# etri/bwa-mem-scale

Hardware: AMD Instinct MI355X
Metric: Mreads/sec through the GPU hot path (seed -> chain -> extend -> dedup, reads and index resident), 150bp SE vs a synthetic genome of GRCh38 size, at 1 MI355X; % HBM roofline in roofline.frac (higher is better)
Workload: dtype int64 intervals / int16 DP (two columns per register; int32 for queries beyond 191 bases or scores beyond 2^14)

## Files before the change

### bwa-mem-scale_amd/csrc/api_chain.hip

```cpp
#include <cstring>
#include <utility>

#include <rocprim/rocprim.hpp>

#include "stage_state.h"

using namespace bwams;

extern "C" {
int bwams_index_set_contigs(bwams_index_t *ix, const bwams_contig_t *contigs, int32_t n_seqs) {
    if (!ix || !contigs || n_seqs <= 0) return BWAMS_ERR_ARG;
    const int64_t l_pac = (ix->fmi.ref_seq_len - 1) / 2;
    int64_t at = 0;
    for (int32_t i = 0; i < n_seqs; ++i) {
        if (contigs[i].offset != at || contigs[i].len <= 0) {
            set_last_error("bwams_index_set_contigs: sequences must tile [0, l_pac) in order");
            return BWAMS_ERR_ARG;
        }
        at += contigs[i].len;
    }
    if (at != l_pac) {
        set_last_error("bwams_index_set_contigs: sequence lengths do not add up to l_pac");
        return BWAMS_ERR_ARG;
    }
    BWAMS_HIP(hipSetDevice(ix->device));
    BWAMS_HIP(ix->d_contigs.alloc((size_t)n_seqs * sizeof(bwams_contig_t)));
    BWAMS_HIP(hipMemcpy(ix->d_contigs.p, contigs, (size_t)n_seqs * sizeof(bwams_contig_t), hipMemcpyHostToDevice));
    ix->n_seqs = n_seqs;
    return BWAMS_OK;
}

static int flt_chained_seeds(bwams_batch *b, StageState *s, const bwams_mem_opt_t *opt, const DevBns &bns) {
    if (!b->idx->fmi.ref) {
        set_last_error("bwams_chain_run: reads of ~1100 bases and more need the .0123 reference (mem_flt_chained_seeds)");
        return BWAMS_ERR_ARG;
    }
    int mx = -128, mn = 127;
    for (int i = 0; i < 25; ++i) { mx = mx > opt->mat[i] ? mx : opt->mat[i]; mn = mn < opt->mat[i] ? mn : opt->mat[i]; }
    if (mx <= 0 || (opt->o_ins + opt->e_ins) + (opt->o_del + opt->e_del) <= mx - mn) {
        set_last_error("bwams_chain_run: the local SW of mem_flt_chained_seeds needs max(mat) > 0 and oe_ins + oe_del > max(mat) - min(mat)");
        return BWAMS_ERR_UNSUPPORTED;
    }
    hipStream_t st = b->stream;
    const int64_t N = s->ch.n_seeds, N1 = N + 1, C = s->ch.n_chains, n1 = s->ch.nseq + 1;
    BWAMS_HIP(s->ext.cnt.ensure((size_t)N1 * 6 * 4)); BWAMS_HIP(s->ext.ewide.ensure((size_t)(N1 > C + 1 ? N1 : C + 1) * 6 * 8));
    BWAMS_HIP(s->ext.eoffs.ensure((size_t)(N1 > C + 1 ? N1 : C + 1) * 6 * 8)); BWAMS_HIP(s->ch.sw_qb.ensure_n((size_t)N1));
    BWAMS_HIP(s->ch.sw_rb.ensure_n((size_t)N1)); BWAMS_HIP(s->ch.sw_read.ensure_n((size_t)N1)); BWAMS_HIP(s->ch.sw_newn.ensure_n((size_t)(C + 1)));
    BWAMS_HIP(s->ch.seeds2.ensure_n((size_t)N1));
    SeedSwArgs W;
    W.chains = s->ch.chains.p; W.n_chains = C; W.seeds = s->ch.seeds.p; W.n_seeds = N; W.enc = b->d_enc.p; W.cum = b->d_cum.p; W.nseq = s->ch.nseq;
    W.ref = b->idx->fmi.ref; W.bns = bns; W.opt = *opt; W.cnt = s->ext.cnt.as<int32_t>(); W.win_qb = s->ch.sw_qb.p; W.win_rb = s->ch.sw_rb.p;
    W.seed_read = s->ch.sw_read.p;
    launch_seedsw_plan(W, s->ext.ewide.as<int64_t>(), st);
    int rc = scan_rows(b, s->ext.ewide.as<int64_t>(), s->ext.eoffs.as<int64_t>(), 3, N1);
    if (rc) return rc;
    int64_t tot[3];
    for (int r = 0; r < 3; ++r) BWAMS_HIP(hipMemcpyAsync(&tot[r], s->ext.eoffs.as<int64_t>() + r * N1 + N, 8, hipMemcpyDeviceToHost, st));
    BWAMS_HIP(hipStreamSynchronize(st));
    if (tot[1] >= ((int64_t)1 << 31) || tot[2] >= ((int64_t)1 << 31)) {
        set_last_error("bwams_chain_run: seed re-scoring buffers exceed the 31-bit offsets of SeqPair; use smaller chunks");
        return BWAMS_ERR_CAPACITY;
    }
    BWAMS_HIP(s->ext.lpairs.ensure_n((size_t)(tot[0] + 1))); BWAMS_HIP(s->ext.lqer.ensure_n((size_t)tot[1] + 64));
    BWAMS_HIP(s->ext.lref.ensure_n((size_t)tot[2] + 64)); BWAMS_HIP(s->ch.sw_res.ensure_n((size_t)(tot[0] + 1)));
    if (tot[0] > 0) {
        launch_seedsw_build(W, s->ext.eoffs.as<int64_t>(), s->ext.lpairs.p, s->ext.lref.p, s->ext.lqer.p, b->cu_count, st);
        SwParams prm;
        sw_params(*opt, 0, &prm);
        (void)launch_ksw(s->ext.lpairs.p, tot[0], s->ext.lref.p, s->ext.lqer.p, prm, 208, 200, s->ch.sw_res.p, b->d_ctr.p, b->cu_count, st);
    }
    int64_t *cw = s->ext.ewide.as<int64_t>();
    int64_t *coff = s->ext.eoffs.as<int64_t>() + 3 * N1;
    launch_seedsw_apply(W, s->ext.eoffs.as<int64_t>(), s->ch.sw_res.p, s->ch.sw_newn.p, cw, st);
    if ((rc = scan_rows(b, cw, coff, 1, C + 1))) return rc;
    int64_t new_total = 0;
    BWAMS_HIP(hipMemcpyAsync(&new_total, coff + C, 8, hipMemcpyDeviceToHost, st));
    launch_seedsw_repack(W, s->ch.sw_newn.p, coff, s->ch.seeds2.p, s->ch.chain_off.as<int64_t>(), s->ch.chain_off.as<int64_t>() + n1, st);
    BWAMS_HIP(hipStreamSynchronize(st));
    std::swap(s->ch.seeds, s->ch.seeds2);
    s->ch.n_seeds = new_total;
    return BWAMS_OK;
}

struct SeedView {
    const bwams_smem_t *smem;
    int64_t n_smem;
    const int64_t *sa_off, *sa_coord;
    int64_t n_sa;
    bool one_smem_quirk;
};
static int chain_common(bwams_batch *b, const bwams_mem_opt_t *opt, const SeedView &sv, int64_t *n_chains, int64_t *n_seeds);

int bwams_chain_run(bwams_batch_t *b, const bwams_mem_opt_t *opt, int64_t *n_chains, int64_t *n_seeds) {
    if (b && b->stages) b->stages->ch.ran = false;
    if (!b || !b->sd.done || !b->sd.with_sa) {
        set_last_error("bwams_chain_run: run bwams_seed_run(with_sa = 1) first");
        return BWAMS_ERR_ARG;
    }
    int rc = check_opt(opt, "bwams_chain_run");
    if (rc) return rc;
    if ((rc = bwams_seed_counts(b, nullptr, nullptr))) return rc;
    SeedView sv;
    sv.smem = b->sd.d_sorted.p; sv.n_smem = b->sd.n_smem; sv.sa_off = b->sd.d_sa_off.p; sv.sa_coord = b->sd.d_sa_coord.p; sv.n_sa = b->sd.n_sa;
    sv.one_smem_quirk = true;
    return chain_common(b, opt, sv, n_chains, n_seeds);
}

int bwams_chain_run_ert(bwams_batch_t *b, const bwams_mem_opt_t *opt, const bwams_ert_mem_t *mems, const int64_t *mem_off,
                        const uint64_t *hits, const int64_t *hit_off, int64_t *n_chains, int64_t *n_seeds) {
    if (b && b->stages) b->stages->ch.ran = false;
    if (!b || b->nseq <= 0 || !mem_off || !hit_off) {
        set_last_error("bwams_chain_run_ert: upload the reads first (bwams_seed_upload) and pass the MEM / hit offsets");
        return BWAMS_ERR_ARG;
    }
    int rc = check_opt(opt, "bwams_chain_run_ert");
    if (rc) return rc;
    const int64_t nseq = b->nseq, n1 = nseq + 1;
    const int64_t n_mems = mem_off[nseq], n_hits = hit_off[nseq];
    if (mem_off[0] != 0 || hit_off[0] != 0 || n_mems < 0 || n_hits < 0 || (n_mems && !mems) || (n_hits && !hits)) return BWAMS_ERR_ARG;
    for (int64_t r = 0; r < nseq; ++r) {
        if (mem_off[r + 1] < mem_off[r] || hit_off[r + 1] < hit_off[r]) { set_last_error("bwams_chain_run_ert: offsets must be non-decreasing"); return BWAMS_ERR_ARG; }
        const int64_t nh = hit_off[r + 1] - hit_off[r];
        for (int64_t i = mem_off[r]; i < mem_off[r + 1]; ++i) {
            const bwams_ert_mem_t &m = mems[i];
            if (m.start < 0 || m.end <= m.start || m.hitcount < 0 || m.hitbeg < 0 || (int64_t)m.hitbeg + m.hitcount > nh) {
                set_last_error("bwams_chain_run_ert: a MEM with an empty span or a hit slice outside its read's hit array");
                return BWAMS_ERR_ARG;
            }
        }
    }
    BWAMS_HIP(hipSetDevice(b->idx->device));
    StageState *s;
    if ((rc = get_state(b, &s))) return rc;
    hipStream_t st = b->stream;
    BWAMS_HIP(s->ch.et_mems.ensure_n((size_t)(n_mems + 1))); BWAMS_HIP(s->ch.et_moff.ensure_n((size_t)n1));
    BWAMS_HIP(s->ch.et_hoff.ensure_n((size_t)n1)); BWAMS_HIP(s->ch.et_hits.ensure_n((size_t)(n_hits + 1)));
    BWAMS_HIP(s->ch.et_smem.ensure_n((size_t)(n_mems + 1))); BWAMS_HIP(s->ch.et_cnt.ensure_n((size_t)(n_mems + 1)));
    BWAMS_HIP(s->ch.et_off.ensure_n((size_t)(n_mems + 1))); BWAMS_HIP(s->ch.et_srt.ensure((size_t)(n_mems + 1) * 24));
    if (n_mems) BWAMS_HIP(hipMemcpyAsync(s->ch.et_mems.p, mems, (size_t)n_mems * sizeof(bwams_ert_mem_t), hipMemcpyHostToDevice, st));
    if (n_hits) BWAMS_HIP(hipMemcpyAsync(s->ch.et_hits.p, hits, (size_t)n_hits * 8, hipMemcpyHostToDevice, st));
    BWAMS_HIP(hipMemcpyAsync(s->ch.et_moff.p, mem_off, (size_t)n1 * 8, hipMemcpyHostToDevice, st));
    BWAMS_HIP(hipMemcpyAsync(s->ch.et_hoff.p, hit_off, (size_t)n1 * 8, hipMemcpyHostToDevice, st));
    ErtArgs E;
    E.mems = s->ch.et_mems.p; E.mem_off = s->ch.et_moff.p; E.hits = s->ch.et_hits.p; E.hit_off = s->ch.et_hoff.p; E.nseq = nseq; E.n_mems = n_mems;
    E.l_pac = (b->idx->fmi.ref_seq_len - 1) / 2; E.max_occ = opt->max_occ; E.pad_ = 0; E.smem_out = s->ch.et_smem.p; E.cnt = s->ch.et_cnt.p;
    E.srt = s->ch.et_srt.p;
    launch_ert_sort(E, st);
    if ((rc = scan_rows(b, s->ch.et_cnt.p, s->ch.et_off.p, 1, n_mems + 1))) return rc;
    int64_t n_sa = 0;
    BWAMS_HIP(hipMemcpyAsync(&n_sa, s->ch.et_off.p + n_mems, 8, hipMemcpyDeviceToHost, st));
    BWAMS_HIP(hipStreamSynchronize(st));
    BWAMS_HIP(s->ch.et_coord.ensure_n((size_t)(n_sa + 1)));
    launch_ert_pick(E, s->ch.et_off.p, s->ch.et_coord.p, st);
    SeedView sv;
    sv.smem = s->ch.et_smem.p; sv.n_smem = n_mems; sv.sa_off = s->ch.et_off.p;
    sv.sa_coord = s->ch.et_coord.p; sv.n_sa = n_sa; sv.one_smem_quirk = false;
    return chain_common(b, opt, sv, n_chains, n_seeds);
}

static int chain_common(bwams_batch *b, const bwams_mem_opt_t *opt, const SeedView &sv, int64_t *n_chains, int64_t *n_seeds) {
    int rc;
    if (b->max_read_len >= 32768) {
        set_last_error("bwams_chain_run: reads of 32768 bases or more are not supported (16-bit query coordinates)");
        return BWAMS_ERR_UNSUPPORTED;
    }
    BWAMS_HIP(hipSetDevice(b->idx->device));
    StageState *s;
    if ((rc = get_state(b, &s))) return rc;
    outdated(s, From::chain);
    hipStream_t st = b->stream;
    const int64_t nseq = b->nseq, n_sa = sv.n_sa, n1 = nseq + 1;
    const size_t ns = (size_t)(n_sa > 0 ? n_sa : 1);
    BWAMS_HIP(s->ch.s_next.ensure_n(ns)); BWAMS_HIP(s->ch.s_ql.ensure_n(ns)); BWAMS_HIP(s->ch.crec.ensure(chain_rec_bytes(n_sa)));
    BWAMS_HIP(s->ch.flt.ensure_n(ns)); BWAMS_HIP(s->ch.f_rec.ensure_n(ns)); BWAMS_HIP(s->ch.f_first.ensure_n(ns));
    BWAMS_HIP(s->ch.f_kept.ensure_n(ns)); BWAMS_HIP(s->ch.f_sel.ensure_n(ns)); BWAMS_HIP(s->ch.n_chn.ensure_n((size_t)n1));
    BWAMS_HIP(s->heavy.ensure_n((size_t)n1)); BWAMS_HIP(s->ch.redo.ensure_n((size_t)n1)); BWAMS_HIP(s->ch.slice.ensure((size_t)n1 * 16));
    BWAMS_HIP(s->ch.okeys.ensure_n((size_t)n1)); BWAMS_HIP(s->ch.okeys2.ensure_n((size_t)n1)); BWAMS_HIP(s->ch.ovals.ensure_n((size_t)n1));
    BWAMS_HIP(s->ch.ovals2.ensure_n((size_t)n1)); BWAMS_HIP(s->ch.nodes.ensure(chain_node_bytes(n_sa, nseq)));
    BWAMS_HIP(s->ch.n_kept.ensure_n((size_t)n1)); BWAMS_HIP(s->ch.n_kept_seeds.ensure_n((size_t)n1)); BWAMS_HIP(s->ch.read_base.ensure_n((size_t)n1));
    BWAMS_HIP(s->ch.frac.ensure_n((size_t)n1)); BWAMS_HIP(s->ch.wide.ensure((size_t)n1 * 16)); BWAMS_HIP(s->ch.chain_off.ensure((size_t)n1 * 16));

    ChainArgs A;
    A.smem = sv.smem; A.n_smem = sv.n_smem; A.sa_off = sv.sa_off; A.sa_coord = sv.sa_coord; A.cum = b->d_cum.p; A.nseq = nseq;
    if ((rc = dev_bns(b->idx, &A.bns))) return rc;
    A.opt = *opt;
    A.s_next = s->ch.s_next.p; A.s_ql = s->ch.s_ql.p; A.crec = s->ch.crec.p; A.flt = s->ch.flt.p; A.f_rec = s->ch.f_rec.p;
    A.f_first = s->ch.f_first.p; A.f_kept = s->ch.f_kept.p; A.f_sel = s->ch.f_sel.p; A.nodes = s->ch.nodes.p; A.n_kept = s->ch.n_kept.p;
    A.n_kept_seeds = s->ch.n_kept_seeds.p; A.n_chn = s->ch.n_chn.p; A.heavy = s->heavy.p; A.redo = s->ch.redo.p; A.slice = s->ch.slice.as<int64_t>();
    A.order = s->ch.ovals2.p; A.read_base = s->ch.read_base.p; A.frac_rep = s->ch.frac.p; A.ctr = b->d_ctr.p; A.seed_batch = knobs().chain_batch;

    BWAMS_HIP(hipEventRecord(s->ev[0], st));
    static_assert(offsetof(DevCounters, dbg) == offsetof(DevCounters, chain_redo) + 4 * sizeof(unsigned long long), "one memset clears chain_redo .. dbg[18]");
    BWAMS_HIP(hipMemsetAsync(&b->d_ctr.p->chain_redo, 0, 23 * sizeof(unsigned long long), st));
    const bool count_ch = knobs().chain_count != 0;
    if (count_ch) BWAMS_HIP(hipMemsetAsync(b->d_ctr.p->dbg + 61, 0, 4 * sizeof(unsigned long long), st));
    BWAMS_HIP(hipMemsetAsync(&b->d_ctr.p->chain_overflow, 0, 29 * sizeof(unsigned long long), st));
    if ((sv.one_smem_quirk ? sv.n_smem <= 1 : sv.n_smem <= 0) || n_sa == 0) {
        BWAMS_HIP(hipMemsetAsync(s->ch.n_kept.p, 0, (size_t)n1 * 4, st));
        BWAMS_HIP(hipMemsetAsync(s->ch.n_kept_seeds.p, 0, (size_t)n1 * 4, st));
    } else {
        launch_chain_count(A, s->ch.okeys.p, s->ch.ovals.p, st);
        if ((rc = with_tmp(b, "bwams_chain_run: radix_sort_pairs_desc", [&](void *tmp, size_t &tb) {
                return rocprim::radix_sort_pairs_desc(tmp, tb, s->ch.okeys.p, s->ch.okeys2.p, s->ch.ovals.p, s->ch.ovals2.p, (size_t)nseq, 0, 32, st);
            }))) return rc;
        if (launch_chain(A, s->ch.okeys.p, b->cu_count, st, s->aux, s->fork, s->join, count_ch)) {
            set_last_error("bwams_chain_run: stream fork/join failed");
            return BWAMS_ERR_DEVICE;
        }
    }
    int64_t tot[2] = {0, 0};
    if (nseq > 0) {
        launch_widen2(A.n_kept, A.n_kept_seeds, nseq, s->ch.wide.as<int64_t>(), st);
        if ((rc = scan_rows(b, s->ch.wide.as<int64_t>(), s->ch.chain_off.as<int64_t>(), 2, n1))) return rc;
        BWAMS_HIP(hipMemcpyAsync(&tot[0], s->ch.chain_off.as<int64_t>() + nseq, 8, hipMemcpyDeviceToHost, st));
        BWAMS_HIP(hipMemcpyAsync(&tot[1], s->ch.chain_off.as<int64_t>() + n1 + nseq, 8, hipMemcpyDeviceToHost, st));
    } else {
        BWAMS_HIP(hipMemsetAsync(s->ch.chain_off.p, 0, (size_t)n1 * 16, st));
    }
    BWAMS_HIP(hipMemcpyAsync(b->h_ctr.p, b->d_ctr.p, sizeof(DevCounters), hipMemcpyDeviceToHost, st));
    BWAMS_HIP(hipStreamSynchronize(st));
    {
        const bool vb = knobs().verbose != 0;
        if (vb) {
            const unsigned long long *d = b->h_ctr.p->dbg;
            fprintf(stderr, "[bwams_chain_run] filter wave tier: reads by chains <=32 %llu <=64 %llu <=128 %llu <=256 %llu <=512 %llu <=960 %llu more %llu (+ %llu taken sequentially by one lane); "
                            "Mcycles: sequential(HBM) %.1f sort %.1f filter %.1f; chains %llu selected %llu; longest read: sort %.2f filter %.2f Mcycles, most chains %llu, most selected %llu\n",
                    d[0], d[1], d[2], d[3], d[4], d[5], d[6], d[18], d[7] / 1e6, d[8] / 1e6, d[9] / 1e6, d[11], d[10], d[12] / 1e6, d[13] / 1e6, d[14], d[15]);
#ifdef BWAMS_CHAINDBG
            static const char *cn[8] = {"XL", "L", "L2", "L1", "M2", "M", "M1", "S"};
            fprintf(stderr, "[bwams_chain_run] chaining wave tier, per class: reads / mean us / longest us / wave-ms:");
            for (int c = 0; c < 8; ++c) fprintf(stderr, "  %s %llu / %.0f / %.0f / %.1f", cn[c], d[32 + 3 * c], d[32 + 3 * c] ? d[33 + 3 * c] * 1e-2 / d[32 + 3 * c] : 0.0, d[34 + 3 * c] * 1e-2, d[33 + 3 * c] * 1e-5);
            fprintf(stderr, "\n");
            fprintf(stderr, "[bwams_chain_run] wave tier phases, G cycles: preamble %.2f chaining %.2f weights+copy %.2f (sort %.2f filter %.2f: all reads); reads %llu seeds %llu; passes %llu settling %llu seeds (%llu new chains), %llu seeds one by one%s; pass parts, G cycles: batch prologue %.2f search %.2f record+test %.2f settle %.2f commit %.2f one-by-one %.2f\n",
                    d[56] / 1e9, d[57] / 1e9, d[58] / 1e9, d[8] / 1e9, d[9] / 1e9, d[59], d[60], count_ch ? d[61] : 0ull, count_ch ? d[63] : 0ull,
                    count_ch ? d[64] : 0ull, count_ch ? d[62] : 0ull, count_ch ? "" : " (these four are counted under BWAMS_CHAIN_COUNT=1 only)", d[65] / 1e9, d[66] / 1e9, d[67] / 1e9, d[68] / 1e9, d[69] / 1e9, d[70] / 1e9);
#endif
        }
    }
    if (b->h_ctr.p->chain_overflow) {
        set_last_error("bwams_chain_run: internal B-tree node region exhausted");
        return BWAMS_ERR_CAPACITY;
    }
    {
        const DevCounters *h = b->h_ctr.p;
        int64_t *c = s->ch.counts;
        for (int i = 0; i < 10; ++i) c[i] = (int64_t)h->chain_class[i];
        c[10] = (int64_t)h->n_heavy; c[11] = (int64_t)h->chain_redo;
        for (int i = 0; i < 7; ++i) c[12 + i] = (int64_t)h->dbg[i];
        c[19] = (int64_t)h->dbg[18];
        c[20] = count_ch ? (int64_t)h->dbg[16] : -1; c[21] = count_ch ? (int64_t)h->dbg[17] : -1;
        c[22] = count_ch ? (int64_t)h->dbg[61] : -1; c[23] = count_ch ? (int64_t)h->dbg[63] : -1;
        c[24] = count_ch ? (int64_t)h->dbg[64] : -1; c[25] = count_ch ? (int64_t)h->dbg[62] : -1;
        s->ch.ran = true;
    }
    const bool has_long = b->h_ctr.p->chain_longread != 0;
    s->ch.n_redo = (int64_t)b->h_ctr.p->chain_redo;
    s->ch.n_chains = tot[0]; s->ch.n_seeds = tot[1]; s->ch.nseq = nseq;
    BWAMS_HIP(s->ch.chains.ensure_n((size_t)(tot[0] + 1))); BWAMS_HIP(s->ch.seeds.ensure_n((size_t)(tot[1] + 1)));
    if (tot[0] > 0) launch_chain_emit(A, s->ch.chain_off.as<int64_t>(), s->ch.chain_off.as<int64_t>() + n1, s->ch.chains.p, s->ch.seeds.p, st);
    if (has_long && tot[0] > 0 && (rc = flt_chained_seeds(b, s, opt, A.bns))) return rc;
    BWAMS_HIP(hipEventRecord(s->ev[1], st));
    BWAMS_HIP(hipGetLastError());
    s->ch.done = true;
    s->opt = *opt;
    if (n_chains) *n_chains = s->ch.n_chains;
    if (n_seeds) *n_seeds = s->ch.n_seeds;
    return BWAMS_OK;
}

int bwams_chain_fetch(bwams_batch_t *b, bwams_chain_t *chains, int64_t chain_cap, bwams_chain_seed_t *seeds,
                      int64_t seed_cap, int64_t *chain_off) {
    if (!b || !b->stages || !b->stages->ch.done) {
        set_last_error("bwams_chain_fetch: no chains on the device");
        return BWAMS_ERR_ARG;
    }
    StageState *s = b->stages;
    if (s->ch.n_chains > chain_cap || s->ch.n_seeds > seed_cap) return BWAMS_ERR_CAPACITY;
    BWAMS_HIP(hipSetDevice(b->idx->device));
    hipStream_t st = b->stream;
    if (s->ch.n_chains) BWAMS_HIP(hipMemcpyAsync(chains, s->ch.chains.p, (size_t)s->ch.n_chains * sizeof(bwams_chain_t), hipMemcpyDeviceToHost, st));
    if (s->ch.n_seeds) BWAMS_HIP(hipMemcpyAsync(seeds, s->ch.seeds.p, (size_t)s->ch.n_seeds * sizeof(bwams_chain_seed_t), hipMemcpyDeviceToHost, st));
    if (chain_off) BWAMS_HIP(hipMemcpyAsync(chain_off, s->ch.chain_off.p, (size_t)(s->ch.nseq + 1) * 8, hipMemcpyDeviceToHost, st));
    BWAMS_HIP(hipStreamSynchronize(st));
    return BWAMS_OK;
}

int bwams_debug_chain_counts(bwams_batch_t *b, int64_t counts[26]) {
    static_assert(kChainCounts == 26, "include/bwams.h documents 26 counters");
    if (!b || !counts || !b->stages || !b->stages->ch.done || !b->stages->ch.ran) {
        set_last_error("bwams_debug_chain_counts: no bwams_chain_run / bwams_chain_run_ert on this batch");
        return BWAMS_ERR_ARG;
    }
    for (int i = 0; i < kChainCounts; ++i) counts[i] = b->stages->ch.counts[i];
    return BWAMS_OK;
}

int bwams_chain_upload(bwams_batch_t *b, const bwams_chain_t *chains, int64_t n_chains, const bwams_chain_seed_t *seeds,
                       int64_t n_seeds, const int64_t *chain_off) {
    if (!b || !chain_off || n_chains < 0 || n_seeds < 0 || (n_chains && (!chains || !seeds))) return BWAMS_ERR_ARG;
    if (b->nseq <= 0) {
        set_last_error("bwams_chain_upload: upload the reads first (bwams_seed_upload)");
        return BWAMS_ERR_ARG;
    }
    const int64_t nseq = b->nseq, n1 = nseq + 1;
    if (chain_off[0] != 0 || chain_off[nseq] != n_chains) return BWAMS_ERR_ARG;
    int64_t at = 0;
    std::string bad;
    int64_t *soff = new int64_t[(size_t)n1];
    for (int64_t r = 0; r < nseq && bad.empty(); ++r) {
        soff[r] = at;
        if (chain_off[r + 1] < chain_off[r]) bad = "chain_off must be non-decreasing";
        for (int64_t j = chain_off[r]; j < chain_off[r + 1] && bad.empty(); ++j) {
            if (chains[j].seqid != r) bad = "chain.seqid does not match chain_off";
            else if (chains[j].seed_off != at || chains[j].n < 0) bad = "chain.seed_off must enumerate the seed array in order";
            at += chains[j].n;
        }
    }
    soff[nseq] = at;
    if (bad.empty() && at != n_seeds) bad = "seed counts do not add up";
    if (!bad.empty()) {
        delete[] soff;
        set_last_error("bwams_chain_upload: " + bad);
        return BWAMS_ERR_ARG;
    }
    BWAMS_HIP(hipSetDevice(b->idx->device));
    StageState *s;
    int rc = get_state(b, &s);
    if (rc) { delete[] soff; return rc; }
    outdated(s, From::chain);
    hipStream_t st = b->stream;
    BWAMS_HIP(s->ch.chain_off.ensure((size_t)n1 * 16)); BWAMS_HIP(s->ch.chains.ensure_n((size_t)(n_chains + 1)));
    BWAMS_HIP(s->ch.seeds.ensure_n((size_t)(n_seeds + 1)));
    BWAMS_HIP(hipMemcpyAsync(s->ch.chain_off.p, chain_off, (size_t)n1 * 8, hipMemcpyHostToDevice, st));
    BWAMS_HIP(hipMemcpyAsync(s->ch.chain_off.as<int64_t>() + n1, soff, (size_t)n1 * 8, hipMemcpyHostToDevice, st));
    if (n_chains) BWAMS_HIP(hipMemcpyAsync(s->ch.chains.p, chains, (size_t)n_chains * sizeof(bwams_chain_t), hipMemcpyHostToDevice, st));
    if (n_seeds) BWAMS_HIP(hipMemcpyAsync(s->ch.seeds.p, seeds, (size_t)n_seeds * sizeof(bwams_chain_seed_t), hipMemcpyHostToDevice, st));
    BWAMS_HIP(hipStreamSynchronize(st));
    delete[] soff;
    s->ch.n_chains = n_chains; s->ch.n_seeds = n_seeds; s->ch.nseq = nseq;
    s->ch.done = true; s->ch.ran = false;
    return BWAMS_OK;
}
}
```

### bwa-mem-scale_amd/csrc/chain.hip

```cpp
#include "common.h"
#include "chain_kernels.h"
#include "wave_ops.h"
#include "ksort.h"

namespace bwams {
namespace {

constexpr int KB_T = 5;
constexpr int KB_MAXK = 2 * KB_T - 1;
constexpr int kLaneSeeds = 32;
constexpr int kLightChains = 16;
struct alignas(16) Node {
    int16_t n, internal;
    int32_t ptr[KB_MAXK + 1];
    int64_t pos[KB_MAXK];
    int32_t key[KB_MAXK];
};
static_assert(sizeof(Node) == 160, "node layout");

struct alignas(16) ChainRec {
    int64_t last_rbeg, endr;
    uint16_t first_qbeg, last_qbeg, last_len, endq;
    int32_t rid, n;
    int32_t first_idx, last_idx;
    int32_t wq, wr;
};
static_assert(sizeof(ChainRec) == 48, "chain record layout");

__host__ __device__ constexpr size_t lds_bytes(int K) { return (size_t)K * (sizeof(ChainRec) + 12) + 64; }
constexpr int kClassS = 128, kClassM1 = 256, kClassM = 512, kClassL1 = 850, kClassL = 1700;
constexpr int kClassM2 = 665, kClassL2 = 1275;
static_assert(lds_bytes(kClassL) <= 160 * 1024, "class L must fit one CU's LDS");
constexpr int kClassXL = 4096;
constexpr int kClassXL2 = 13000;
__host__ __device__ constexpr size_t lds_bytes_xl(int K) { return (size_t)K * 12 + 64; }

struct RidCache { int64_t lo, hi; int rid; };

__device__ __forceinline__ int pos2rid(const DevBns &b, int64_t pos_f, RidCache &rc) {
    if (pos_f >= b.l_pac) return -1;
    if (pos_f >= rc.lo && pos_f < rc.hi) return rc.rid;
    const int mid = pos2rid(b, pos_f);
    const int64_t off = b.contigs[mid].offset;
    if (pos_f >= off) { rc.lo = off; rc.hi = mid == b.n_seqs - 1 ? b.l_pac : b.contigs[mid + 1].offset; rc.rid = mid; }
    return mid;
}
__device__ __forceinline__ int intv2rid(const DevBns &b, int64_t rb, int64_t re, RidCache &rc) {
    if (rb < b.l_pac && re > b.l_pac) return -2;
    const int rid_b = pos2rid(b, depos(b, rb), rc);
    const int rid_e = rb < re ? pos2rid(b, depos(b, re - 1), rc) : rid_b;
    return rid_b == rid_e ? rid_b : -1;
}

struct WaveBns { int64_t off; };
__device__ __forceinline__ WaveBns wave_bns_load(const DevBns &b, int lane) {
    WaveBns w;
    const int stride = b.n_seqs <= 64 ? 1 : 64;
    const int64_t i = (int64_t)lane * stride;
    w.off = i < b.n_seqs ? b.contigs[i].offset : INT64_MAX;
    return w;
}
__device__ __forceinline__ int pos2rid_w(const DevBns &b, const WaveBns &w, int64_t pos_f, int lane) {
    if (pos_f >= b.l_pac) return -1;
    const int c = __popcll(__ballot(w.off <= pos_f)) - 1;
    if (b.n_seqs <= 64) return c;
    const int i = c * 64 + lane;
    const int64_t o = i < b.n_seqs ? b.contigs[i].offset : INT64_MAX;
    return c * 64 + __popcll(__ballot(o <= pos_f)) - 1;
}
__device__ __forceinline__ int intv2rid_w(const DevBns &b, const WaveBns &w, int64_t rb, int64_t re, int lane) {
    if (rb < b.l_pac && re > b.l_pac) return -2;
    const int rid_b = pos2rid_w(b, w, depos(b, rb), lane);
    const int rid_e = rb < re ? pos2rid_w(b, w, depos(b, re - 1), lane) : rid_b;
    return rid_b == rid_e ? rid_b : -1;
}

struct ReadCtx {
    Node *nodes;
    ChainRec *crec;
    int32_t n_nodes, cap_nodes, root;
    int32_t n_keys;
    bool overflow;
    bool wr;
};

__device__ __forceinline__ int32_t new_node(ReadCtx &c) {
    if (c.n_nodes >= c.cap_nodes) { c.overflow = true; return 0; }
    if (c.wr) { Node *x = &c.nodes[c.n_nodes]; x->n = 0; x->internal = 0; }
    return c.n_nodes++;
}

struct NodeR {
    int32_t n, internal;
    int64_t pos[KB_MAXK];
    int32_t key[KB_MAXK];
    int32_t ptr[KB_MAXK + 1];
};
__device__ __forceinline__ void load_node(const Node *p, NodeR &x, bool want_ptr) {
    x.n = p->n; x.internal = p->internal;
#pragma unroll
    for (int t = 0; t < KB_MAXK; ++t) { x.pos[t] = p->pos[t]; x.key[t] = p->key[t]; }
#pragma unroll
    for (int t = 0; t <= KB_MAXK; ++t) x.ptr[t] = want_ptr ? (int32_t)p->ptr[t] : 0;
}

__device__ __forceinline__ int node_search(const NodeR &x, int64_t k, bool &eq) {
    int cnt = 0;
    bool e = false;
#pragma unroll
    for (int t = 0; t < KB_MAXK; ++t)
        if (t < x.n) { cnt += x.pos[t] < k ? 1 : 0; e |= x.pos[t] == k; }
    eq = e;
    return e ? cnt : cnt - 1;
}
__device__ __forceinline__ int32_t sel_key(const NodeR &x, int i) {
    int32_t v = x.key[0];
#pragma unroll
    for (int t = 1; t < KB_MAXK; ++t) v = i == t ? x.key[t] : v;
    return v;
}
__device__ __forceinline__ int64_t sel_pos(const NodeR &x, int i) {
    int64_t v = x.pos[0];
#pragma unroll
    for (int t = 1; t < KB_MAXK; ++t) v = i == t ? x.pos[t] : v;
    return v;
}
__device__ __forceinline__ int32_t sel_ptr(const NodeR &x, int i) {
    int32_t v = x.ptr[0];
#pragma unroll
    for (int t = 1; t <= KB_MAXK; ++t) v = i == t ? x.ptr[t] : v;
    return v;
}

__device__ __forceinline__ int32_t kbt_lower(const ReadCtx &c, int64_t k, int64_t &lower_pos) {
    int32_t lower = -1, xi = c.root;
    for (;;) {
        NodeR x;
        load_node(&c.nodes[xi], x, true);
        bool eq;
        const int i = node_search(x, k, eq);
        if (i >= 0) { lower = sel_key(x, i); lower_pos = sel_pos(x, i); }
        if (i >= 0 && eq) return lower;
        if (!x.internal) return lower;
        xi = sel_ptr(x, i + 1);
    }
}

__device__ __forceinline__ void kbt_split(ReadCtx &c, int32_t xi, int i, int32_t yi) {
    const int32_t zi = new_node(c);
    if (c.overflow || !c.wr) return;
    Node *x = &c.nodes[xi], *y = &c.nodes[yi], *z = &c.nodes[zi];
    z->internal = y->internal;
    z->n = KB_T - 1;
    for (int t = 0; t < KB_T - 1; ++t) { z->key[t] = y->key[KB_T + t]; z->pos[t] = y->pos[KB_T + t]; }
    if (y->internal) for (int t = 0; t < KB_T; ++t) z->ptr[t] = y->ptr[KB_T + t];
    y->n = KB_T - 1;
    const int xn = x->n;
    for (int t = xn; t > i; --t) x->ptr[t + 1] = x->ptr[t];
    x->ptr[i + 1] = zi;
    for (int t = xn - 1; t >= i; --t) { x->key[t + 1] = x->key[t]; x->pos[t + 1] = x->pos[t]; }
    x->key[i] = y->key[KB_T - 1];
    x->pos[i] = y->pos[KB_T - 1];
    x->n = (int16_t)(xn + 1);
}

__device__ __forceinline__ void kbt_put(ReadCtx &c, int32_t id, int64_t k) {
    ++c.n_keys;
    int32_t xi = c.root;
    if (c.nodes[xi].n == KB_MAXK) {
        const int32_t s = new_node(c);
        if (c.overflow) return;
        if (c.wr) { c.nodes[s].internal = 1; c.nodes[s].n = 0; c.nodes[s].ptr[0] = xi; }
        c.root = s;
        kbt_split(c, s, 0, xi);
        if (c.overflow) return;
        xi = s;
    }
    for (;;) {
        Node *px = &c.nodes[xi];
        NodeR x;
        load_node(px, x, true);
        bool eq;
        if (!x.internal) {
            const int i = node_search(x, k, eq);
            if (c.wr) {
#pragma unroll
                for (int t = KB_MAXK - 1; t >= 1; --t)
                    if (t > i + 1 && t <= x.n) { px->key[t] = x.key[t - 1]; px->pos[t] = x.pos[t - 1]; }
#pragma unroll
                for (int t = 0; t < KB_MAXK; ++t)
                    if (t == i + 1) { px->key[t] = id; px->pos[t] = k; }
                px->n = (int16_t)(x.n + 1);
            }
            return;
        }
        int i = node_search(x, k, eq) + 1;
        int32_t ci = sel_ptr(x, i);
        if (c.nodes[ci].n == KB_MAXK) {
            const int64_t median = c.nodes[ci].pos[KB_T - 1];
            kbt_split(c, xi, i, ci);
            if (c.overflow) return;
            if (k > median) ci = c.nodes[xi].ptr[i + 1];
        }
        xi = ci;
    }
}

struct WPath { int32_t leaf; int16_t slot, n; bool ok; };

__device__ __forceinline__ int32_t kbt_traverse(const ReadCtx &c, int32_t *out) {
    int32_t sx[16];
    int32_t si[16];
    int sp = 0, n = 0;
    sx[0] = c.root; si[0] = 0;
    while (sp >= 0) {
        const Node *x = &c.nodes[sx[sp]];
        if (!x->internal) {
            for (int t = 0; t < x->n; ++t) { if (c.wr) out[n] = x->key[t]; ++n; }
            --sp;
            continue;
        }
        const int i = si[sp];
        if (i > 0 && i - 1 < x->n) { if (c.wr) out[n] = x->key[i - 1]; ++n; }
        if (i <= x->n && sp < 15) {
            si[sp] = i + 1;
            ++sp;
            sx[sp] = x->ptr[i]; si[sp] = 0;
        } else --sp;
    }
    return n;
}

struct FltLt { __device__ __forceinline__ bool operator()(const uint2 &a, const uint2 &b) const { return a.x > b.x; } };

struct FltClose {
    __device__ __forceinline__ void operator()(uint2 *a, int n, void *scratch, int lane, FltLt) const {
        uint2 *out = reinterpret_cast<uint2 *>(scratch);
        if (n > 64) {
            unsigned long long *key = reinterpret_cast<unsigned long long *>(scratch);
            out = reinterpret_cast<uint2 *>(key + n);
            for (int x = lane; x < n; x += 64) key[x] = ((unsigned long long)(0x7fffffffu - a[x].x) << 32) | (unsigned long long)(unsigned)x;
            __syncthreads();
            int P = 128;
            while (P < n) P <<= 1;
            for (int k = 2; k <= P; k <<= 1) {
                for (int j = k >> 1; j > 0; j >>= 1) {
                    const bool flip = j == (k >> 1);
                    for (int c0 = 0; c0 < (P >> 1); c0 += 64) {
                        const int c = c0 + lane;
                        const int i = ((c & ~(j - 1)) << 1) | (c & (j - 1));
                        const int l = flip ? (i ^ (k - 1)) : i + j;
                        if (l < n) {
                            const unsigned long long x = key[i], y = key[l];
                            if (y < x) { key[i] = y; key[l] = x; }
                        }
                    }
                    __syncthreads();
                }
            }
            for (int x = lane; x < n; x += 64) out[x] = a[(uint32_t)key[x]];
            __syncthreads();
        } else {
            const int x = lane;
            const uint2 v = x < n ? a[x] : make_uint2(0u, 0u);
            int pos = 0;
            for (int y = 0; y < n; ++y) {
                const uint32_t wy = a[y].x;
                pos += (wy > v.x || (wy == v.x && y < x)) ? 1 : 0;
            }
            if (x < n) out[pos] = v;
            __syncthreads();
        }
        for (int x = lane; x < n; x += 64) a[x] = out[x];
        __syncthreads();
    }
};

__device__ __forceinline__ void wave_flt_sort(uint2 *a, int n, void *scratch, int lane, int depth0 = 0) {
    wave_ks_introsort(a, n, scratch, reinterpret_cast<int *>(reinterpret_cast<char *>(scratch) + (size_t)n * 8), lane, FltLt(), FltClose(), depth0);
}

__device__ void filter_seq(const bwams_mem_opt_t &opt, int n_chn, uint4 *rec, int32_t *kept, int32_t *sel) {
    int n_sel = 0;
    kept[0] = 3;
    sel[n_sel++] = 0;
    for (int i = 1; i < n_chn; ++i) {
        bool large_ovlp = false;
        const uint4 ri = rec[i];
        const int bi = (int)ri.x, ei = (int)ri.y, wi = (int)(ri.z & 0x7fffffffu);
        const bool alt_i = (ri.z >> 31) != 0;
        int k;
        for (k = 0; k < n_sel; ++k) {
            const int j = sel[k];
            const uint4 rj = rec[j];
            const int bj = (int)rj.x, ej = (int)rj.y;
            const int b_max = bj > bi ? bj : bi;
            const int e_min = ej < ei ? ej : ei;
            const bool alt_j = (rj.z >> 31) != 0;
            if (e_min > b_max && (!alt_j || alt_i)) {
                const int li = ei - bi, lj = ej - bj;
                const int min_l = li < lj ? li : lj;
                if ((float)(e_min - b_max) >= (float)min_l * opt.mask_level && min_l < opt.max_chain_gap) {
                    large_ovlp = true;
                    if ((int)rj.w < 0) rec[j].w = (uint32_t)i;
                    const int wj = (int)(rj.z & 0x7fffffffu);
                    if ((float)wi < (float)wj * opt.drop_ratio && wj - wi >= (opt.min_seed_len << 1)) break;
                }
            }
        }
        if (k == n_sel) {
            sel[n_sel++] = i;
            kept[i] = large_ovlp ? 2 : 3;
        }
    }
    for (int i = 0; i < n_sel; ++i) {
        const int f = (int)rec[sel[i]].w;
        if (f >= 0) kept[f] = 1;
    }
}

__device__ void finish_read(const ChainArgs &A, int64_t r, int64_t base, int n_chn, int L) {
    uint2 *fl = A.flt + base;
    uint4 *rec = A.f_rec + base;
    int32_t *kept = A.f_kept + base, *first = A.f_first + base;
    const ChainRec *crec = reinterpret_cast<const ChainRec *>(A.crec) + base;
    int i, k;
    for (i = k = 0; i < n_chn; ++i) {
        if (kept[i] == 0 || kept[i] == 3) continue;
        if (++k >= A.opt.max_chain_extend) break;
    }
    for (; i < n_chn; ++i)
        if (kept[i] < 3) kept[i] = 0;
    int n_seeds = 0;
    for (i = k = 0; i < n_chn; ++i) {
        if (kept[i] == 0) continue;
        const uint2 f = fl[i];
        const uint32_t alt = rec[i].z & 0x80000000u;
        fl[k] = make_uint2(f.x | ((unsigned)kept[i] << 29) | alt, f.y);
        first[k] = (int32_t)rec[i].w;
        n_seeds += crec[f.y].n;
        ++k;
    }
    A.n_kept[r] = k;
    A.n_kept_seeds[r] = n_seeds;
    if (k) {
        const double min_l = A.opt.min_chain_weight ? (double)(1.1f * (float)A.opt.min_chain_weight) : (double)5.5f * log((double)L);
        if (!(min_l > (double)(0.05f * (float)L))) atomicAdd(&A.ctr->chain_longread, 1ull);
    }
}

__device__ __forceinline__ uint4 make_rec(const ChainArgs &A, const ChainRec &c, uint32_t w) {
    const uint32_t alt = A.bns.contigs[c.rid].is_alt != 0 ? 0x80000000u : 0u;
    return make_uint4((uint32_t)c.first_qbeg, (uint32_t)(c.last_qbeg + c.last_len), w | alt, 0xffffffffu);
}

#ifndef BWAMS_CHAIN_COUNT_TU
__global__ void chain_slice_kernel(ChainArgs A) {
    const int64_t i = (int64_t)blockIdx.x * blockDim.x + threadIdx.x;
    if (i >= A.n_smem) return;
    const int64_t r = (int64_t)A.smem[i].rid;
    if (i == 0 || (int64_t)A.smem[i - 1].rid != r) A.slice[2 * r] = i;
    if (i + 1 == A.n_smem || (int64_t)A.smem[i + 1].rid != r) A.slice[2 * r + 1] = i + 1;
}
__global__ void chain_count_kernel(ChainArgs A, uint32_t *keys, uint32_t *vals) {
    const int64_t r = (int64_t)blockIdx.x * blockDim.x + threadIdx.x;
    const bool live = r < A.nseq;
    int64_t cnt = 0;
    if (live) {
        const int64_t beg = A.slice[2 * r], end = A.slice[2 * r + 1];
        cnt = beg < end ? A.sa_off[end] - A.sa_off[beg] : 0;
        keys[r] = (uint32_t)(cnt < 0xffffffffll ? cnt : 0xffffffffll);
        vals[r] = (uint32_t)r;
    }
    const int thr[10] = {kClassL, kClassL1, kClassM, kClassM1, kClassS, kLaneSeeds, kClassXL, kClassL2, kClassM2, kClassXL2};
    if (!__ballot(live && cnt > kLaneSeeds)) return;
#pragma unroll
    for (int c = 0; c < 10; ++c) {
        const unsigned long long m = __ballot(live && cnt > thr[c]);
        if (m && (threadIdx.x & 63) == 0) atomicAdd(&A.ctr->chain_class[c], (unsigned long long)__popcll(m));
    }
}

#endif

__device__ __forceinline__ int sarr_lower(const int64_t *key, int n, int64_t k, int lane, bool &eq) {
    int base = 0;
    if (n > 4096) {
        const int nsc = (n + 4095) >> 12;
        const unsigned long long ms = __ballot(lane < nsc && key[lane << 12] <= k);
        if (!ms) { eq = false; return -1; }
        base = (__popcll(ms) - 1) << 12;
        key += base;
        n = n - base < 4096 ? n - base : 4096;
    }
    const int nch = (n + 63) >> 6;
    const unsigned long long mc = __ballot(lane < nch && key[lane << 6] <= k);
    if (!mc) { eq = false; return -1; }
    const int c = __popcll(mc) - 1;
    const int i = (c << 6) + lane;
    const int64_t my = i < n ? key[i] : 0;
    const unsigned long long mk = __ballot(i < n && my <= k);
    const int idx = base + (c << 6) + __popcll(mk) - 1;
    eq = __ballot(i < n && my == k) != 0;
    return idx;
}
__device__ __forceinline__ void sarr_insert(int64_t *key, int32_t *cid, int n, int at, int64_t k, int32_t id, int lane) {
    for (int base = ((n - at) >> 6) << 6; base >= 0; base -= 64) {
        const int i = at + base + lane;
        const bool mv = i < n;
        const int64_t kk = mv ? key[i] : 0;
        const int32_t cc = mv ? cid[i] : 0;
        if (mv) { key[i + 1] = kk; cid[i + 1] = cc; }
    }
    if (lane == 0) { key[at] = k; cid[at] = id; }
}

struct SeedCtx {
    bool crec_hbm;
    const int64_t *pos;
    int32_t *s_next;
    int2 *s_ql;
    ChainRec *crec;
    int64_t *s_key;
    int32_t *s_cid;
};
__device__ __forceinline__ bool chain_seed_one(const ChainArgs &A, const SeedCtx &S, int &n_keys, int32_t g, int64_t rbeg, int rid, int qbeg,
                                               int slen, int lane) {
    const bool wr = lane == 0;
    const int64_t l_pac = A.bns.l_pac;
    bool to_add = true, eq = false;
    int idx = -1;
    if (n_keys) {
        idx = sarr_lower(S.s_key, n_keys, rbeg, lane, eq);
        if (idx >= 0) {
            const int32_t lower = S.s_cid[idx];
            const int64_t fr = S.s_key[idx];
            ChainRec ch = S.crec[lower];
            const int64_t lr = ch.last_rbeg;
            const int64_t qend = ch.last_qbeg + ch.last_len, rend = lr + ch.last_len;
            if (rid != ch.rid) to_add = true;
            else if (qbeg >= ch.first_qbeg && qbeg + slen <= qend && rbeg >= fr && rbeg + slen <= rend) to_add = false;
            else if ((lr < l_pac || fr < l_pac) && rbeg >= l_pac) to_add = true;
            else {
                const int64_t x = qbeg - ch.last_qbeg, y = rbeg - lr;
                if (y >= 0 && x - y <= A.opt.w && y - x <= A.opt.w && x - ch.last_len < A.opt.max_chain_gap && y - ch.last_len < A.opt.max_chain_gap) {
                    if (wr) { S.s_ql[g] = make_int2(qbeg, slen); S.s_next[g] = -1; S.s_next[ch.last_idx] = g; }
                    if (qbeg >= ch.endq) ch.wq += slen; else if (qbeg + slen > ch.endq) ch.wq += qbeg + slen - ch.endq;
                    ch.endq = (uint16_t)((int)ch.endq > qbeg + slen ? (int)ch.endq : qbeg + slen);
                    if (rbeg >= ch.endr) ch.wr += slen; else if (rbeg + slen > ch.endr) ch.wr += (int)(rbeg + slen - ch.endr);
                    ch.endr = ch.endr > rbeg + slen ? ch.endr : rbeg + slen;
                    ch.last_rbeg = rbeg; ch.last_qbeg = (uint16_t)qbeg; ch.last_len = (uint16_t)slen; ch.last_idx = g; ch.n += 1;
                    if (wr) S.crec[lower] = ch;
                    to_add = false;
                }
            }
        }
    }
    if (to_add) {
        if (n_keys && eq) return false;
        if (wr) {
            S.s_ql[g] = make_int2(qbeg, slen); S.s_next[g] = -1;
            ChainRec ch;
            ch.last_rbeg = rbeg; ch.endr = rbeg + slen;
            ch.first_qbeg = (uint16_t)qbeg; ch.last_qbeg = (uint16_t)qbeg; ch.last_len = (uint16_t)slen; ch.endq = (uint16_t)(qbeg + slen);
            ch.rid = rid; ch.n = 1; ch.first_idx = g; ch.last_idx = g; ch.wq = slen; ch.wr = slen;
            S.crec[n_keys] = ch;
        }
        sarr_insert(S.s_key, S.s_cid, n_keys, n_keys ? idx + 1 : 0, rbeg, n_keys, lane);
        ++n_keys;
    }
    return true;
}
template <bool COUNT>
__device__ bool chain_seeds_batch(const ChainArgs &A, const SeedCtx &S, int &n_keys, const bwams_smem_t *sm, int64_t beg, int64_t end, int64_t base,
                                  int32_t cnt, RidCache &rc, const WaveBns &wb, int lane) {
    enum { NONE = 0, NOOP = 1, MERGE = 2, NEW = 3, UNSETTLED = 4 };
    const int64_t l_pac = A.bns.l_pac;
    const unsigned long long below = (1ull << lane) - 1ull;
    const int w = A.opt.w, max_gap = A.opt.max_chain_gap;
    int64_t i_lo = beg;
#ifdef BWAMS_CHAINDBG
    unsigned long long tq[6] = {0, 0, 0, 0, 0, 0};
    unsigned long long tq0 = __builtin_amdgcn_s_memtime();
#define TQ(k) { const unsigned long long t_ = __builtin_amdgcn_s_memtime(); tq[k] += t_ - tq0; tq0 = t_; }
#else
#define TQ(k)
#endif
    const int nsm = (int)(end - beg);
    const bool sm_regs = nsm <= 64;
    int sm_start = INT32_MAX, sm_q = 0, sm_l = 0;
    if (sm_regs && lane < nsm) {
        sm_start = (int)(A.sa_off[beg + lane] - base);
        sm_q = (int)sm[beg + lane].m; sm_l = (int)sm[beg + lane].n + 1 - sm_q;
    }
    for (int32_t gb = 0; gb < cnt; gb += 64) {
        const int32_t g = gb + lane;
        bool pend = g < cnt;
        const int64_t rbeg = pend ? S.pos[g] : 0;
        int qbeg = 0, slen = 0;
        if (sm_regs) {
            int k = 0;
            for (int i = 0; i < nsm; ++i) k += __builtin_amdgcn_readlane(sm_start, i) <= g ? 1 : 0;
            const int src = k > 0 ? k - 1 : 0;
            qbeg = __shfl(sm_q, src); slen = __shfl(sm_l, src);
        } else {
            int64_t lo = i_lo, hi = end - 1;
            if (pend) {
                while (lo < hi) {
                    const int64_t mid = (lo + hi + 1) >> 1;
                    if (A.sa_off[mid] - base <= g) lo = mid; else hi = mid - 1;
                }
                qbeg = (int)sm[lo].m; slen = (int)sm[lo].n + 1 - qbeg;
            }
            i_lo = readlane64(lo, 0);
        }
        int rid = -1;
        if (A.bns.n_seqs <= 64) {
            const int64_t rb = rbeg, re = rbeg + slen;
            const int64_t pb = depos(A.bns, rb), pe = rb < re ? depos(A.bns, re - 1) : pb;
            int cb = 0, ce = 0;
            for (int i = 0; i < A.bns.n_seqs; ++i) {
                const int64_t o = readlane64(wb.off, i);
                cb += o <= pb ? 1 : 0; ce += o <= pe ? 1 : 0;
            }
            rid = (rb < l_pac && re > l_pac) ? -2 : cb == ce ? cb - 1 : -1;
        } else if (pend) rid = intv2rid(A.bns, rbeg, rbeg + slen, rc);
        pend = pend && rid >= 0;
        int one_by_one = 0;
        unsigned long long mp;
        TQ(0)
        while ((mp = __ballot(pend)) != 0ull) {
            if (one_by_one) {
                const int l0 = __builtin_ctzll(mp);
                if (!chain_seed_one(A, S, n_keys, gb + l0, readlane64(rbeg, l0), __builtin_amdgcn_readlane(rid, l0), __builtin_amdgcn_readlane(qbeg, l0),
                                    __builtin_amdgcn_readlane(slen, l0), lane)) return false;
                if (lane == l0) pend = false;
                if constexpr (COUNT) { if (lane == 0) atomicAdd(&A.ctr->dbg[62], 1ull); }
                --one_by_one;
                TQ(5)
                continue;
            }
            const int n = n_keys;
            int idx = -1;
            if (n) {
                int step = 1;
                while ((step << 1) <= n) step <<= 1;
                for (; step > 0; step >>= 1) {
                    const int t = idx + step;
                    if (pend && t < n && S.s_key[t] <= rbeg) idx = t;
                }
            }
            TQ(1)
            int64_t lo_key = INT64_MIN;
            int32_t lower = -1;
            int act = NONE;
            ChainRec ch;
            ch.last_rbeg = 0; ch.endr = 0; ch.first_qbeg = ch.last_qbeg = ch.last_len = ch.endq = 0; ch.rid = ch.n = ch.first_idx = ch.last_idx = ch.wq = ch.wr = 0;
            if (pend) {
                act = NEW;
                if (idx >= 0) {
                    lo_key = S.s_key[idx];
                    lower = S.s_cid[idx];
                    ch = S.crec[lower];
                    const int64_t lr = ch.last_rbeg;
                    const int64_t qend = ch.last_qbeg + ch.last_len, rend = lr + ch.last_len;
                    if (rid != ch.rid) act = NEW;
                    else if (qbeg >= ch.first_qbeg && qbeg + slen <= qend && rbeg >= lo_key && rbeg + slen <= rend) act = NOOP;
                    else if ((lr < l_pac || lo_key < l_pac) && rbeg >= l_pac) act = NEW;
                    else {
                        const int64_t x = qbeg - ch.last_qbeg, y = rbeg - lr;
                        if (y >= 0 && x - y <= w && y - x <= w && x - ch.last_len < max_gap && y - ch.last_len < max_gap) act = MERGE;
                    }
                }
            }
            const bool eq = pend && idx >= 0 && lo_key == rbeg;
            TQ(2)
            int64_t best = lo_key;
            int best_rid = -1, best_q = 0, best_l = 0;
            bool displaced = false, touched = false;
            int first_open = 64;
            bool shared = false;
            {
                unsigned *mark = reinterpret_cast<unsigned *>(S.s_cid);
                const bool in_arr = pend && idx >= 0;
                if (in_arr) atomicAdd(&mark[idx], 1u << 24);
                if (in_arr) shared = (mark[idx] >> 24) > 1u;
                if (in_arr) atomicSub(&mark[idx], 1u << 24);
                const bool under = pend && idx < 0;
                const int n_under = __popcll(__ballot(under));
                if (under && n_under > 1) shared = true;
            }
            unsigned long long rem = __ballot(pend && shared);
            while (rem) {
                const int i = __builtin_ctzll(rem);
                rem &= rem - 1;
                int fin = act;
                if (displaced) {
                    const int64_t x = qbeg - best_q, y = rbeg - best;
                    if (rid != best_rid) fin = NEW;
                    else if (qbeg >= best_q && qbeg + slen <= best_q + best_l && rbeg + slen <= best + best_l) fin = NOOP;
                    else if (best < l_pac && rbeg >= l_pac) fin = NEW;
                    else fin = (x - y <= w && y - x <= w && x - best_l < max_gap && y - best_l < max_gap) ? UNSETTLED : NEW;
                } else if (touched) fin = UNSETTLED;
                const int a_i = __builtin_amdgcn_readlane(fin, i);
                if (a_i == UNSETTLED) { first_open = i; break; }
                if (lane == i) act = fin;
                if (a_i == NEW) {
                    const int64_t rb_i = readlane64(rbeg, i);
                    const int rid_i = __builtin_amdgcn_readlane(rid, i), q_i = __builtin_amdgcn_readlane(qbeg, i), l_i = __builtin_amdgcn_readlane(slen, i);
                    if (lane > i && rb_i <= rbeg && rb_i > best) { best = rb_i; best_rid = rid_i; best_q = q_i; best_l = l_i; displaced = true; }
                } else if (a_i == MERGE) {
                    const int low_i = __builtin_amdgcn_readlane(lower, i);
                    if (lane > i && lower == low_i) touched = true;
                }
            }
            const bool com = pend && lane < first_open;
            TQ(3)
            const unsigned long long m_new = __ballot(com && act == NEW);
            if (__ballot(com && act == NEW && (eq || (displaced && best == rbeg)))) return false;
            if (com && act == MERGE) {
                S.s_ql[g] = make_int2(qbeg, slen); S.s_next[g] = -1; S.s_next[ch.last_idx] = g;
                if (qbeg >= ch.endq) ch.wq += slen; else if (qbeg + slen > ch.endq) ch.wq += qbeg + slen - ch.endq;
                ch.endq = (uint16_t)((int)ch.endq > qbeg + slen ? (int)ch.endq : qbeg + slen);
                if (rbeg >= ch.endr) ch.wr += slen; else if (rbeg + slen > ch.endr) ch.wr += (int)(rbeg + slen - ch.endr);
                ch.endr = ch.endr > rbeg + slen ? ch.endr : rbeg + slen;
                ch.last_rbeg = rbeg; ch.last_qbeg = (uint16_t)qbeg; ch.last_len = (uint16_t)slen; ch.last_idx = g; ch.n += 1;
                S.crec[lower] = ch;
            }
            if (m_new) {
                const int m = __popcll(m_new);
                const bool mine = com && act == NEW;
                int min_idx = mine ? idx : n;
                for (int d = 32; d >= 1; d >>= 1) { const int o = __shfl_xor(min_idx, d); min_idx = o < min_idx ? o : min_idx; }
                for (int cb = n > 0 ? ((n - 1) >> 6) << 6 : -64; cb >= 0 && cb + 63 > min_idx; cb -= 64) {
                    const int p = cb + lane;
                    const bool mv = p < n;
                    const int64_t kk = mv ? S.s_key[p] : 0;
                    const int32_t cc = mv ? S.s_cid[p] : 0;
                    int sh = __popcll(__ballot(mine && idx < cb));
                    unsigned long long mm = __ballot(mine && idx >= cb && idx < cb + 64);
                    while (mm) { const int i = __builtin_ctzll(mm); mm &= mm - 1; sh += __builtin_amdgcn_readlane(idx, i) < p ? 1 : 0; }
                    if (mv && sh) { S.s_key[p + sh] = kk; S.s_cid[p + sh] = cc; }
                }
                int rank = 0;
                { unsigned long long mm = m_new; while (mm) { const int i = __builtin_ctzll(mm); mm &= mm - 1; rank += __builtin_amdgcn_readlane(idx, i) < idx ? 1 : 0; } }
                { unsigned long long mm = m_new & __ballot(shared); while (mm) { const int i = __builtin_ctzll(mm); mm &= mm - 1; rank += (__builtin_amdgcn_readlane(idx, i) == idx && readlane64(rbeg, i) < rbeg) ? 1 : 0; } }
                if (mine) {
                    const int32_t cid = n + __popcll(m_new & below);
                    S.s_ql[g] = make_int2(qbeg, slen); S.s_next[g] = -1;
                    ChainRec nc;
                    nc.last_rbeg = rbeg; nc.endr = rbeg + slen;
                    nc.first_qbeg = (uint16_t)qbeg; nc.last_qbeg = (uint16_t)qbeg; nc.last_len = (uint16_t)slen; nc.endq = (uint16_t)(qbeg + slen);
                    nc.rid = rid; nc.n = 1; nc.first_idx = g; nc.last_idx = g; nc.wq = slen; nc.wr = slen;
                    S.crec[cid] = nc;
                    S.s_key[idx + 1 + rank] = rbeg; S.s_cid[idx + 1 + rank] = cid;
                }
                n_keys = n + m;
            }
            if (com) pend = false;
            if constexpr (COUNT) {
                const unsigned long long n_com = (unsigned long long)__popcll(__ballot(com));
                if (lane == 0) { atomicAdd(&A.ctr->dbg[61], 1ull); atomicAdd(&A.ctr->dbg[63], n_com); atomicAdd(&A.ctr->dbg[64], (unsigned long long)__popcll(m_new)); }
            }
            if (__popcll(__ballot(com)) <= 1) one_by_one = 8;
            if (S.crec_hbm) __threadfence_block();
            TQ(4)
        }
    }
#ifdef BWAMS_CHAINDBG
    if (lane == 0) for (int k = 0; k < 6; ++k) atomicAdd(&A.ctr->dbg[65 + k], tq[k]);
#endif
    return true;
}

__device__ void heavy_read(const ChainArgs &A, int64_t r, int64_t base, int n_chn, unsigned char *lds, int cap, int lane);
__host__ __device__ constexpr size_t heavy_lds_bytes(int cap);
template <bool LDS, int CONT = 0, bool CREC_HBM = false, bool COUNT = false>
__device__ __forceinline__ bool chain_read(const ChainArgs &A, int64_t r, int lane, int nl, Node *nodes, int32_t cap_nodes,
                                           ChainRec *crec_w, int32_t cap_chains) {
    const bool wr = lane == 0;
#ifdef BWAMS_CHAINDBG
    const unsigned long long tp0 = __builtin_amdgcn_s_memtime();
#endif
    if (wr) {
        A.n_kept[r] = 0;
        A.n_kept_seeds[r] = 0;
        A.read_base[r] = 0;
        A.n_chn[r] = 0;
    }
    const bwams_smem_t *sm = A.smem;
    const int64_t beg = A.slice[2 * r], end = A.slice[2 * r + 1];
    const int L = (int)(A.cum[r + 1] - A.cum[r]);
    if (beg == end || L < A.opt.min_seed_len) return true;

    int b = 0, e = 0, l_rep = 0;
    if (nl == 64 && end - beg <= 64) {
        const bool has = beg + lane < end;
        const int my_b = has ? (int)sm[beg + lane].m : 0, my_e = has ? (int)sm[beg + lane].n + 1 : 0;
        unsigned long long rep = __ballot(has && sm[beg + lane].s > (int64_t)A.opt.max_occ);
        while (rep) {
            const int i = __builtin_ctzll(rep);
            rep &= rep - 1;
            const int sb = __builtin_amdgcn_readlane(my_b, i), se = __builtin_amdgcn_readlane(my_e, i);
            if (sb > e) { l_rep += e - b; b = sb; e = se; }
            else e = e > se ? e : se;
        }
    } else
    for (int64_t i = beg; i < end; ++i) {
        const int sb = (int)sm[i].m, se = (int)sm[i].n + 1;
        if (sm[i].s <= (int64_t)A.opt.max_occ) continue;
        if (sb > e) { l_rep += e - b; b = sb; e = se; }
        else e = e > se ? e : se;
    }
    l_rep += e - b;
    if (wr) A.frac_rep[r] = (float)l_rep / (float)L;

    const int64_t base = A.sa_off[beg];
    const int32_t cnt = (int32_t)(A.sa_off[end] - base);
    if (wr) A.read_base[r] = base;
    if (cnt == 0) return true;
    const int64_t *pos = A.sa_coord + base;
    int32_t *s_next = A.s_next + base;
    int2 *s_ql = A.s_ql + base;
    ChainRec *crec_g = reinterpret_cast<ChainRec *>(A.crec) + base;
    ChainRec *crec;
    ReadCtx c;
    if constexpr (LDS) {
        crec = CREC_HBM ? crec_g : crec_w;
        c.nodes = nodes; c.cap_nodes = cap_nodes;
    } else {
        crec = crec_g;
        const int64_t nbase = (base >> 1) + 2 * r;
        c.nodes = reinterpret_cast<Node *>(A.nodes) + nbase;
        c.cap_nodes = (int32_t)((((base + cnt) >> 1) + 2 * (r + 1)) - nbase);
    }
    c.crec = crec;
    c.n_nodes = 0; c.n_keys = 0; c.overflow = false; c.wr = wr;
    int64_t *s_key = nullptr;
    int32_t *s_cid = nullptr;
    if constexpr (CONT == 1) {
        s_key = reinterpret_cast<int64_t *>(nodes);
        s_cid = reinterpret_cast<int32_t *>(s_key + cap_chains);
    } else c.root = new_node(c);
    RidCache rc;
    rc.lo = 0; rc.hi = -1; rc.rid = 0;
    WaveBns wb;
    wb.off = 0;
    if (nl == 64 && A.bns.n_seqs <= 4096) wb = wave_bns_load(A.bns, lane);
    if (LDS && cnt > cap_chains) { if (wr) atomicAdd(&A.ctr->chain_overflow, 1ull); return true; }

    const int64_t l_pac = A.bns.l_pac;
#ifdef BWAMS_CHAINDBG
    const unsigned long long tp1 = __builtin_amdgcn_s_memtime();
#endif
    if constexpr (CONT == 1) {
        if (nl == 64 && A.seed_batch) {
            SeedCtx S;
            S.pos = pos; S.s_next = s_next; S.s_ql = s_ql; S.crec = crec; S.s_key = s_key; S.s_cid = s_cid; S.crec_hbm = CREC_HBM;
            int nk = 0;
            if (!chain_seeds_batch<COUNT>(A, S, nk, sm, beg, end, base, cnt, rc, wb, lane)) return false;
            c.n_keys = nk;
        }
    }
    if (!(CONT == 1 && nl == 64 && A.seed_batch))
    for (int64_t i = beg; i < end; ++i) {
        const int qbeg = (int)sm[i].m, slen = (int)sm[i].n + 1 - (int)sm[i].m;
        const int32_t g0 = (int32_t)(A.sa_off[i] - base), g1 = (int32_t)(A.sa_off[i + 1] - base);
        int64_t pos64 = 0;
        for (int32_t g = g0; g < g1; ++g) {
            int64_t rbeg;
            if (nl == 64) {
                const int j = (g - g0) & 63;
                if (j == 0) pos64 = g + lane < g1 ? pos[g + lane] : 0;
                rbeg = (int64_t)(((unsigned long long)(uint32_t)__builtin_amdgcn_readlane((int)(pos64 >> 32), j) << 32) |
                                 (unsigned long long)(uint32_t)__builtin_amdgcn_readlane((int)pos64, j));
            } else rbeg = pos[g];
            const int rid = nl == 64 && A.bns.n_seqs <= 4096 ? intv2rid_w(A.bns, wb, rbeg, rbeg + slen, lane)
                                                               : intv2rid(A.bns, rbeg, rbeg + slen, rc);
            if (rid < 0) continue;
            bool to_add = true;
            WPath path;
            path.ok = false;
            if (c.n_keys) {
                int64_t fr = 0;
                int32_t lower;
                if constexpr (CONT == 1) {
                    bool eq;
                    const int idx = sarr_lower(s_key, c.n_keys, rbeg, lane, eq);
                    lower = -1;
                    if (idx >= 0) { lower = s_cid[idx]; fr = s_key[idx]; }
                    path.slot = (int16_t)0; path.leaf = idx; path.ok = !eq;
                } else lower = kbt_lower(c, rbeg, fr);
                if (lower >= 0) {
                    ChainRec ch = crec[lower];
                    const int64_t lr = ch.last_rbeg;
                    const int64_t qend = ch.last_qbeg + ch.last_len, rend = lr + ch.last_len;
                    if (rid != ch.rid) to_add = true;
                    else if (qbeg >= ch.first_qbeg && qbeg + slen <= qend && rbeg >= fr && rbeg + slen <= rend) to_add = false;
                    else if ((lr < l_pac || fr < l_pac) && rbeg >= l_pac) to_add = true;
                    else {
                        const int64_t x = qbeg - ch.last_qbeg, y = rbeg - lr;
                        if (y >= 0 && x - y <= A.opt.w && y - x <= A.opt.w && x - ch.last_len < A.opt.max_chain_gap &&
                            y - ch.last_len < A.opt.max_chain_gap) {
                            if (wr) {
                                s_ql[g] = make_int2(qbeg, slen);
                                s_next[g] = -1;
                                s_next[ch.last_idx] = g;
                            }
                            if (qbeg >= ch.endq) ch.wq += slen; else if (qbeg + slen > ch.endq) ch.wq += qbeg + slen - ch.endq;
                            ch.endq = (uint16_t)((int)ch.endq > qbeg + slen ? (int)ch.endq : qbeg + slen);
                            if (rbeg >= ch.endr) ch.wr += slen; else if (rbeg + slen > ch.endr) ch.wr += (int)(rbeg + slen - ch.endr);
                            ch.endr = ch.endr > rbeg + slen ? ch.endr : rbeg + slen;
                            ch.last_rbeg = rbeg; ch.last_qbeg = (uint16_t)qbeg; ch.last_len = (uint16_t)slen; ch.last_idx = g; ch.n += 1;
                            if (wr) crec[lower] = ch;
                            to_add = false;
                        }
                    }
                }
            }
            if (to_add) {
                if (wr) { s_ql[g] = make_int2(qbeg, slen); s_next[g] = -1; }
                ChainRec ch;
                ch.last_rbeg = rbeg; ch.endr = rbeg + slen;
                ch.first_qbeg = (uint16_t)qbeg; ch.last_qbeg = (uint16_t)qbeg; ch.last_len = (uint16_t)slen; ch.endq = (uint16_t)(qbeg + slen);
                ch.rid = rid; ch.n = 1; ch.first_idx = g; ch.last_idx = g; ch.wq = slen; ch.wr = slen;
                const int32_t cid = c.n_keys;
                if (wr) crec[cid] = ch;
                if constexpr (CONT == 1) {
                    if (c.n_keys && !path.ok) return false;
                    sarr_insert(s_key, s_cid, c.n_keys, c.n_keys ? path.leaf + 1 : 0, rbeg, cid, lane);
                    ++c.n_keys;
                } else kbt_put(c, cid, rbeg);
                if (c.overflow) { if (wr) atomicAdd(&A.ctr->chain_overflow, 1ull); return true; }
            }
        }
    }
    if (c.n_keys == 0) return true;
#ifdef BWAMS_CHAINDBG
    const unsigned long long tp2 = __builtin_amdgcn_s_memtime();
#endif

    int32_t *ord = A.f_first + base;
    int32_t n_trav;
    if constexpr (CONT == 1) {
        n_trav = c.n_keys;
        for (int32_t t = lane; t < n_trav; t += nl) ord[t] = s_cid[t];
        __threadfence_block();
    } else n_trav = kbt_traverse(c, ord);
    uint2 *fl = A.flt + base;
    int n_chn = 0;
    if (nl == 64) {
        uint2 first = make_uint2(0u, 0u);
        for (int32_t t0 = 0; t0 < n_trav; t0 += 64) {
            const int32_t t = t0 + lane;
            const bool ok = t < n_trav;
            int32_t id = 0;
            if (ok) { if constexpr (CONT == 1) id = s_cid[t]; else id = ord[t]; }
            const ChainRec *pc = &crec[id];
            int w = pc->wr < pc->wq ? pc->wr : pc->wq;
            w = w < (1 << 30) ? w : (1 << 30) - 1;
            if (t0 == 0) first = make_uint2((unsigned)__builtin_amdgcn_readfirstlane(w), (unsigned)__builtin_amdgcn_readfirstlane(id));
            const bool keep = ok && w >= A.opt.min_chain_weight;
            const unsigned long long m = __ballot(keep);
            if (keep) fl[n_chn + __popcll(m & ((1ull << lane) - 1ull))] = make_uint2((unsigned)w, (unsigned)id);
            n_chn += __popcll(m);
        }
        if (n_chn == 0 && wr) fl[0] = first;
        __threadfence_block();
    } else
    for (int32_t t = 0; t < n_trav; ++t) {
        const int32_t id = ord[t];
        const ChainRec ch = crec[id];
        int w = ch.wr < ch.wq ? ch.wr : ch.wq;
        w = w < (1 << 30) ? w : (1 << 30) - 1;
        if (t == 0 && wr) fl[0] = make_uint2((unsigned)w, (unsigned)id);
        if (w < A.opt.min_chain_weight) continue;
        if (wr) fl[n_chn] = make_uint2((unsigned)w, (unsigned)id);
        ++n_chn;
    }
    if (n_chn == 0) n_chn = 1;
    if constexpr (LDS && !CREC_HBM)
        for (int32_t k = lane; k < c.n_keys; k += nl) crec_g[k] = crec_w[k];
    if constexpr (LDS) {
        if (nl == 64) {
#ifdef BWAMS_CHAINDBG
            if (wr) {
                const unsigned long long tp3 = __builtin_amdgcn_s_memtime();
                atomicAdd(&A.ctr->dbg[56], tp1 - tp0); atomicAdd(&A.ctr->dbg[57], tp2 - tp1); atomicAdd(&A.ctr->dbg[58], tp3 - tp2);
                atomicAdd(&A.ctr->dbg[59], 1ull); atomicAdd(&A.ctr->dbg[60], (unsigned long long)cnt);
            }
#endif
            unsigned char *region = CREC_HBM ? reinterpret_cast<unsigned char *>(nodes) : reinterpret_cast<unsigned char *>(crec_w);
            const size_t bytes = (size_t)cap_chains * (CREC_HBM ? 12 : sizeof(ChainRec) + 12);
            const int cap_f = (int)((bytes - 64) / 41);
            if (cap_f >= 64 && n_chn <= cap_f) {
                if (wr) A.n_chn[r] = n_chn;
                __threadfence_block();
                if constexpr (COUNT) { if (wr) atomicAdd(&A.ctr->dbg[16], 1ull); }
                heavy_read(A, r, base, n_chn, region, cap_f, lane);
                return true;
            }
        }
    }
    if (!wr) return true;
    A.n_chn[r] = n_chn;
    if (n_chn > kLightChains) {
        const unsigned long long slot = atomicAdd(&A.ctr->n_heavy, 1ull);
        A.heavy[slot] = (int32_t)r;
        return true;
    }
    if constexpr (COUNT) atomicAdd(&A.ctr->dbg[17], 1ull);
    ks_introsort(fl, n_chn, FltLt());
    uint4 *rec = A.f_rec + base;
    int32_t *kept = A.f_kept + base;
    for (int i = 0; i < n_chn; ++i) {
        rec[i] = make_rec(A, crec[fl[i].y], fl[i].x);
        kept[i] = 0;
    }
    filter_seq(A.opt, n_chn, rec, kept, A.f_sel + base);
    if constexpr (LDS) __threadfence_block();
    finish_read(A, r, base, n_chn, L);
    return true;
}

template <bool COUNT>
__global__ __launch_bounds__(64) void chain_kernel(ChainArgs A, const uint32_t *__restrict__ n_seeds) {
    const int64_t r = (int64_t)blockIdx.x * blockDim.x + threadIdx.x;
    if (r >= A.nseq) return;
    if (n_seeds[r] > (uint32_t)kLaneSeeds) return;
    chain_read<false, 0, false, COUNT>(A, r, 0, 1, nullptr, 0, nullptr, 0);
}

template <bool COUNT>
__global__ __launch_bounds__(64) __attribute__((amdgpu_waves_per_eu(3, 3))) void chain_wave_kernel(ChainArgs A, const unsigned long long *lo_p, const unsigned long long *hi_p,
                                                        unsigned long long *ticket, int K) {
    extern __shared__ __align__(16) unsigned char l_mem[];
    const int lane = threadIdx.x;
    const int64_t lo = lo_p ? (int64_t)*lo_p : 0, hi = (int64_t)*hi_p;
    ChainRec *l_crec = reinterpret_cast<ChainRec *>(l_mem);
    Node *l_nodes = reinterpret_cast<Node *>(l_mem + (size_t)(K > 0 ? K : 0) * sizeof(ChainRec));
    for (;;) {
        const unsigned long long t = wave_ticket(ticket, 1ull);
        if (lo + (int64_t)t >= hi) break;
        const int64_t r = (int64_t)A.order[lo + (int64_t)t];
#ifdef BWAMS_CHAINDBG
        const unsigned long long tk0 = wall_clock64();
#endif
        if (K < 0) {
            if (!chain_read<true, 1, true, COUNT>(A, r, lane, 64, reinterpret_cast<Node *>(l_mem), 0, nullptr, -K) && lane == 0)
                A.redo[atomicAdd(&A.ctr->chain_redo, 1ull)] = (int32_t)r;
        } else if (K) {
            if (!chain_read<true, 1, false, COUNT>(A, r, lane, 64, l_nodes, 0, l_crec, K) && lane == 0)
                A.redo[atomicAdd(&A.ctr->chain_redo, 1ull)] = (int32_t)r;
        } else chain_read<false, 0, false, COUNT>(A, r, lane, 64, nullptr, 0, nullptr, 0);
        __syncthreads();
#ifdef BWAMS_CHAINDBG
        if (lane == 0) {
            const int c = K < 0 ? 0 : K == kClassL ? 1 : K == kClassL2 ? 2 : K == kClassL1 ? 3 : K == kClassM2 ? 4 : K == kClassM ? 5 : K == kClassM1 ? 6 : 7;
            const unsigned long long dt = wall_clock64() - tk0;
            atomicAdd(&A.ctr->dbg[32 + 3 * c], 1ull); atomicAdd(&A.ctr->dbg[33 + 3 * c], dt); atomicMax(&A.ctr->dbg[34 + 3 * c], dt);
        }
#endif
    }
}

template <bool COUNT>
__global__ __launch_bounds__(64) void chain_redo_kernel(ChainArgs A) {
    const int lane = threadIdx.x;
    const int64_t n = (int64_t)A.ctr->chain_redo;
    for (;;) {
        const int64_t t = (int64_t)wave_ticket(&A.ctr->chain_redo_ticket, 1ull);
        if (t >= n) break;
        chain_read<false, 0, false, COUNT>(A, A.redo[t], lane, 64, nullptr, 0, nullptr, 0);
    }
}

constexpr int kHeavyCap[6] = {64, 128, 256, 512, 960, 3840};
__host__ __device__ constexpr size_t heavy_lds_bytes(int cap) { return (size_t)cap * 41 + 64; }
static_assert(heavy_lds_bytes(kHeavyCap[5]) <= 160 * 1024, "the largest class must fit one CU's LDS");
static_assert(160 * 1024 / 41 <= 65535, "wave_ks_introsort's stopper lists are uint16_t: no LDS class may hold more chains");

__device__ void heavy_read(const ChainArgs &A, int64_t r, int64_t base, int n_chn, unsigned char *lds, int cap, int lane) {
    uint4 *l_rec = reinterpret_cast<uint4 *>(lds);
    uint4 *l_sel = l_rec + cap;
    uint2 *l_fl = reinterpret_cast<uint2 *>(l_sel + cap);
    uint8_t *l_kept = reinterpret_cast<uint8_t *>(l_fl + cap);
    const int L = (int)(A.cum[r + 1] - A.cum[r]);
    uint2 *fl = A.flt + base;
    const ChainRec *crec = reinterpret_cast<const ChainRec *>(A.crec) + base;
    const unsigned long long t_0 = __builtin_amdgcn_s_memtime();
    if (lane == 0) {
        const int bk = n_chn <= 32 ? 0 : n_chn <= 64 ? 1 : n_chn <= 128 ? 2 : n_chn <= 256 ? 3 : n_chn <= 512 ? 4 : n_chn <= 960 ? 5 : 6;
        atomicAdd(&A.ctr->dbg[bk], 1ull);
    }
    {
        __syncthreads();
        for (int i = lane; i < n_chn; i += 64) l_fl[i] = fl[i];
        __syncthreads();
        wave_flt_sort(l_fl, n_chn, l_sel, lane);
        const unsigned long long t_1 = __builtin_amdgcn_s_memtime();
        for (int i = lane; i < n_chn; i += 64) {
            const uint2 f = l_fl[i];
            l_rec[i] = make_rec(A, crec[f.y], f.x);
            l_kept[i] = 0;
        }
        __syncthreads();
        int n_sel = 1;
        if (lane == 0) { const uint4 r0 = l_rec[0]; l_sel[0] = make_uint4(r0.x, r0.y, r0.z, 0u); l_kept[0] = 3; }
        __syncthreads();
        const float mask_level = A.opt.mask_level, drop_ratio = A.opt.drop_ratio;
        const int max_gap = A.opt.max_chain_gap, min_dw = A.opt.min_seed_len << 1;
        for (int ib = 1; ib < n_chn; ib += 64) {
            const int i = ib + lane;
            const bool valid = i < n_chn;
            const uint4 ri = valid ? l_rec[i] : make_uint4(0, 0, 0, 0);
            const int bi = (int)ri.x, ei = (int)ri.y, wi = (int)(ri.z & 0x7fffffffu), li = ei - bi;
            const bool alt_i = (ri.z >> 31) != 0;
            const float fwi = (float)wi;
            bool alive = valid, large = false;
            const int n_sel0 = n_sel;
            for (int k0 = 0; k0 < n_sel0; k0 += 4) {
                uint4 rj[4];
#pragma unroll
                for (int u = 0; u < 4; ++u) rj[u] = l_sel[k0 + u < n_sel0 ? k0 + u : n_sel0 - 1];
#pragma unroll
                for (int u = 0; u < 4; ++u) {
                    if (k0 + u >= n_sel0) break;
                    const int bj = (int)rj[u].x, ej = (int)rj[u].y;
                    const int b_max = bj > bi ? bj : bi, e_min = ej < ei ? ej : ei;
                    const bool alt_j = (rj[u].z >> 31) != 0;
                    const int lj = ej - bj, min_l = li < lj ? li : lj;
                    const bool lg = alive && e_min > b_max && (!alt_j || alt_i) && (float)(e_min - b_max) >= (float)min_l * mask_level && min_l < max_gap;
                    const unsigned long long m_lg = __ballot(lg);
                    if (m_lg) {
                        if (lane == __builtin_ctzll(m_lg)) atomicMin(&l_rec[rj[u].w].w, (uint32_t)i);
                        if (lg) {
                            large = true;
                            const int wj = (int)(rj[u].z & 0x7fffffffu);
                            if (fwi < (float)wj * drop_ratio && wj - wi >= min_dw) alive = false;
                        }
                    }
                }
                if (!__ballot(alive)) break;
            }
            unsigned long long todo = __ballot(alive);
            while (todo) {
                const int lp = __builtin_ctzll(todo);
                const int bj = __builtin_amdgcn_readlane(bi, lp), ej = __builtin_amdgcn_readlane(ei, lp);
                const uint32_t zj = (uint32_t)__builtin_amdgcn_readlane((int)ri.z, lp);
                if (lane == lp) { l_sel[n_sel] = make_uint4(ri.x, ri.y, ri.z, (uint32_t)i); l_kept[i] = large ? 2 : 3; }
                ++n_sel;
                const int b_max = bj > bi ? bj : bi, e_min = ej < ei ? ej : ei;
                const bool alt_j = (zj >> 31) != 0;
                const int lj = ej - bj, min_l = li < lj ? li : lj;
                const bool lg = alive && lane > lp && e_min > b_max && (!alt_j || alt_i) && (float)(e_min - b_max) >= (float)min_l * mask_level && min_l < max_gap;
                const unsigned long long m_lg = __ballot(lg);
                if (m_lg) {
                    if (lane == __builtin_ctzll(m_lg)) l_rec[ib + lp].w = (uint32_t)i;
                    if (lg) {
                        large = true;
                        const int wj = (int)(zj & 0x7fffffffu);
                        if (fwi < (float)wj * drop_ratio && wj - wi >= min_dw) alive = false;
                    }
                }
                todo = __ballot(alive) & ~((2ull << lp) - 1ull);
            }
            __syncthreads();
        }
        for (int k = lane; k < n_sel; k += 64) {
            const int f = (int)l_rec[l_sel[k].w].w;
            if (f >= 0) l_kept[f] = 1;
        }
        __syncthreads();
        if (lane == 0) {
            const unsigned long long t_2 = __builtin_amdgcn_s_memtime();
            atomicAdd(&A.ctr->dbg[8], t_1 - t_0);
            atomicAdd(&A.ctr->dbg[9], t_2 - t_1);
            atomicMax(&A.ctr->dbg[12], t_1 - t_0);
            atomicMax(&A.ctr->dbg[13], t_2 - t_1);
            atomicMax(&A.ctr->dbg[14], (unsigned long long)n_chn);
            atomicMax(&A.ctr->dbg[15], (unsigned long long)n_sel);
            atomicAdd(&A.ctr->dbg[10], (unsigned long long)n_sel);
            atomicAdd(&A.ctr->dbg[11], (unsigned long long)n_chn);
        }
        if (A.opt.max_chain_extend <= n_chn) {
            if (lane == 0) {
                int i, k;
                for (i = k = 0; i < n_chn; ++i) {
                    if (l_kept[i] == 0 || l_kept[i] == 3) continue;
                    if (++k >= A.opt.max_chain_extend) break;
                }
                for (; i < n_chn; ++i)
                    if (l_kept[i] < 3) l_kept[i] = 0;
            }
            __syncthreads();
        }
        int32_t *first = A.f_first + base;
        int n_out = 0, n_seeds = 0;
        for (int ib = 0; ib < n_chn; ib += 64) {
            const int i = ib + lane;
            const int kp = i < n_chn ? (int)l_kept[i] : 0;
            const unsigned long long m = __ballot(kp != 0);
            if (kp) {
                const int o = n_out + __popcll(m & ((1ull << lane) - 1ull));
                const uint2 f = l_fl[i];
                const uint4 rc4 = l_rec[i];
                fl[o] = make_uint2(f.x | ((unsigned)kp << 29) | (rc4.z & 0x80000000u), f.y);
                first[o] = (int32_t)rc4.w;
                n_seeds += crec[f.y].n;
            }
            n_out += __popcll(m);
        }
        for (int d = 32; d >= 1; d >>= 1) n_seeds += __shfl_xor(n_seeds, d);
        if (lane == 0) {
            A.n_kept[r] = n_out;
            A.n_kept_seeds[r] = n_seeds;
            if (n_out) {
                const double min_l = A.opt.min_chain_weight ? (double)(1.1f * (float)A.opt.min_chain_weight) : (double)5.5f * log((double)L);
                if (!(min_l > (double)(0.05f * (float)L))) atomicAdd(&A.ctr->chain_longread, 1ull);
            }
        }
        __syncthreads();
    }
}

__global__ __launch_bounds__(64) void chain_heavy_kernel(ChainArgs A, const unsigned long long *n_heavy_p, int cap_lo, int cap,
                                                         unsigned long long *ticket) {
    extern __shared__ __align__(16) unsigned char l_heavy[];
    const int kLdsChains = cap;
    const int lane = threadIdx.x;
    const int64_t n_heavy = (int64_t)*n_heavy_p;
    for (;;) {
        const int64_t hi = (int64_t)wave_ticket(ticket, 1ull);
        if (hi >= n_heavy) break;
        const int64_t r = A.heavy[hi];
        const int64_t base = A.read_base[r];
        const int n_chn = A.n_chn[r];
        if (n_chn <= cap_lo || (n_chn > cap && cap != kHeavyCap[5])) continue;
        const int L = (int)(A.cum[r + 1] - A.cum[r]);
        uint2 *fl = A.flt + base;
        uint4 *rec = A.f_rec + base;
        int32_t *kept = A.f_kept + base;
        const ChainRec *crec = reinterpret_cast<const ChainRec *>(A.crec) + base;
        if (n_chn > kLdsChains) {
            const unsigned long long t_0 = __builtin_amdgcn_s_memtime();
            if (lane == 0) {
                atomicAdd(&A.ctr->dbg[18], 1ull);
                ks_introsort(fl, n_chn, FltLt());
                for (int i = 0; i < n_chn; ++i) { rec[i] = make_rec(A, crec[fl[i].y], fl[i].x); kept[i] = 0; }
                filter_seq(A.opt, n_chn, rec, kept, A.f_sel + base);
                finish_read(A, r, base, n_chn, L);
                atomicAdd(&A.ctr->dbg[7], __builtin_amdgcn_s_memtime() - t_0);
            }
            continue;
        }
        heavy_read(A, r, base, n_chn, l_heavy, cap, lane);
    }
}

#ifndef BWAMS_CHAIN_COUNT_TU
__global__ __launch_bounds__(256) void chain_emit_kernel(ChainArgs A, const int64_t *__restrict__ chain_off, const int64_t *__restrict__ seed_off,
                                                         bwams_chain_t *chains, bwams_chain_seed_t *seeds) {
    const int64_t r = ((int64_t)blockIdx.x * blockDim.x + threadIdx.x) >> 4;
    const int sub = threadIdx.x & 15;
    const bool live = r < A.nseq;
    const int nk = live ? A.n_kept[r] : 0;
    if (nk == 0) return;
    const int64_t base = A.read_base[r];
    const uint2 *fl = A.flt + base;
    const int32_t *first = A.f_first + base;
    const int32_t *s_next = A.s_next + base;
    const int2 *s_ql = A.s_ql + base;
    const int64_t *pos = A.sa_coord + base;
    const ChainRec *crec = reinterpret_cast<const ChainRec *>(A.crec) + base;
    int64_t so0 = seed_off[r];
    const int64_t co = chain_off[r];
    const float frac = A.frac_rep[r];
    for (int j0 = 0; j0 < nk; j0 += 16) {
        const int j = j0 + sub;
        const bool has = j < nk;
        uint2 f = make_uint2(0u, 0u);
        ChainRec ch;
        ch.n = 0; ch.first_idx = -1; ch.rid = 0;
        if (has) { f = fl[j]; ch = crec[f.y]; }
        const int n = has ? ch.n : 0;
        int incl = n;
        for (int d = 1; d < 16; d <<= 1) {
            const int o = __shfl_up(incl, d, 16);
            if (sub >= d) incl += o;
        }
        const int total = __shfl(incl, 15, 16);
        if (has) {
            int64_t so = so0 + (incl - n);
            bwams_chain_t c;
            c.seqid = (int32_t)r; c.cseed = 0;
            c.n = n;
            int m = 1;
            while (m < n) m <<= 1;
            c.m = m;
            c.first = first[j];
            c.rid = ch.rid;
            c.w_kept_alt = f.x;
            c.frac_rep = frac;
            c.pos = pos[ch.first_idx];
            c.seed_off = so;
            chains[co + j] = c;
            for (int32_t g = ch.first_idx; g >= 0; g = s_next[g]) {
                bwams_chain_seed_t sd;
                sd.rbeg = pos[g];
                sd.qbeg = s_ql[g].x; sd.len = s_ql[g].y; sd.score = sd.len;
                sd.done = 0; sd.pad0_[0] = sd.pad0_[1] = sd.pad0_[2] = 0;
                sd.aln = 0; sd.pad1_ = 0;
                seeds[so++] = sd;
            }
        }
        so0 += total;
    }
}

constexpr int kFltTestN = 1024;
__global__ __launch_bounds__(64) void flt_sort_test_kernel(const uint2 *__restrict__ in, int n, int mode, int32_t *__restrict__ order,
                                                           uint2 *__restrict__ scratch) {
    __shared__ uint2 l_a[kFltTestN];
    __shared__ uint4 l_scr[kFltTestN];
    const int lane = threadIdx.x;
    if (mode == 2 || mode == 4) {
        for (int i = lane; i < n; i += 64) scratch[i] = in[i];
        __syncthreads();
        if (lane == 0) ks_introsort(scratch, n, FltLt(), mode == 4 ? 2 : 0);
        __syncthreads();
        for (int i = lane; i < n; i += 64) order[i] = (int32_t)scratch[i].y;
        return;
    }
    for (int i = lane; i < n; i += 64) l_a[i] = in[i];
    __syncthreads();
    wave_flt_sort(l_a, n, l_scr, lane, mode == 3 ? 2 : 0);
    for (int i = lane; i < n; i += 64) order[i] = (int32_t)l_a[i].y;
}

#endif

}

#ifndef BWAMS_CHAIN_COUNT_TU
size_t chain_node_bytes(int64_t n_sa, int64_t nseq) { return (size_t)((n_sa >> 1) + 2 * nseq + 4) * sizeof(Node); }
size_t chain_rec_bytes(int64_t n_sa) { return (size_t)(n_sa > 0 ? n_sa : 1) * sizeof(ChainRec); }

void launch_chain_count(const ChainArgs &A, uint32_t *keys, uint32_t *vals, hipStream_t st) {
    if (A.nseq <= 0) return;
    (void)hipMemsetAsync(A.slice, 0, (size_t)A.nseq * 16, st);
    if (A.n_smem > 0) chain_slice_kernel<<<(unsigned)((A.n_smem + 255) / 256), 256, 0, st>>>(A);
    chain_count_kernel<<<(unsigned)((A.nseq + 255) / 256), 256, 0, st>>>(A, keys, vals);
}
#endif
template <bool COUNT>
static int launch_chain_t(const ChainArgs &A, const uint32_t *n_seeds, int cu_count, hipStream_t st, hipStream_t *aux,
                          hipEvent_t fork, hipEvent_t *join) {
    if (A.nseq <= 0) return 0;
    unsigned long long *cls = A.ctr->chain_class, *tk = A.ctr->chain_ticket;
    if (hipFuncSetAttribute(reinterpret_cast<const void *>(chain_wave_kernel<COUNT>), hipFuncAttributeMaxDynamicSharedMemorySize,
                            (int)lds_bytes_xl(kClassXL2)) != hipSuccess) return -1;
    if (hipEventRecord(fork, st) != hipSuccess) return -1;
    for (int i = 0; i < 7; ++i)
        if (hipStreamWaitEvent(aux[i], fork, 0) != hipSuccess) return -1;
    chain_wave_kernel<COUNT><<<(unsigned)cu_count, 64, lds_bytes_xl(kClassXL2), st>>>(A, cls + 9, cls + 6, tk + 9, -kClassXL2);
    chain_wave_kernel<COUNT><<<(unsigned)(cu_count * 8), 64, 0, aux[0]>>>(A, nullptr, cls + 9, tk + 0, 0);
    chain_wave_kernel<COUNT><<<(unsigned)cu_count, 64, lds_bytes_xl(kClassXL), aux[0]>>>(A, cls + 6, cls + 0, tk + 6, -kClassXL);
    chain_wave_kernel<COUNT><<<(unsigned)cu_count, 64, lds_bytes(kClassL), aux[1]>>>(A, cls + 0, cls + 7, tk + 1, kClassL);
    chain_wave_kernel<COUNT><<<(unsigned)(cu_count * 2), 64, lds_bytes(kClassL2), aux[5]>>>(A, cls + 7, cls + 1, tk + 7, kClassL2);
    chain_wave_kernel<COUNT><<<(unsigned)(cu_count * 3), 64, lds_bytes(kClassL1), aux[2]>>>(A, cls + 1, cls + 8, tk + 2, kClassL1);
    chain_wave_kernel<COUNT><<<(unsigned)(cu_count * 4), 64, lds_bytes(kClassM2), aux[6]>>>(A, cls + 8, cls + 2, tk + 8, kClassM2);
    chain_wave_kernel<COUNT><<<(unsigned)(cu_count * 8), 64, lds_bytes(kClassM1), aux[2]>>>(A, cls + 3, cls + 4, tk + 4, kClassM1);
    chain_wave_kernel<COUNT><<<(unsigned)(cu_count * 12), 64, lds_bytes(kClassS), aux[3]>>>(A, cls + 4, cls + 5, tk + 5, kClassS);
    chain_kernel<COUNT><<<(unsigned)((A.nseq + 63) / 64), 64, 0, aux[1]>>>(A, n_seeds);
    chain_wave_kernel<COUNT><<<(unsigned)(cu_count * 5), 64, lds_bytes(kClassM), aux[5]>>>(A, cls + 2, cls + 3, tk + 3, kClassM);
    for (int i = 0; i < 7; ++i) {
        if (hipEventRecord(join[i], aux[i]) != hipSuccess) return -1;
        if (hipStreamWaitEvent(st, join[i], 0) != hipSuccess) return -1;
    }
    chain_redo_kernel<COUNT><<<(unsigned)(cu_count * 2), 64, 0, st>>>(A);
    if (hipFuncSetAttribute(reinterpret_cast<const void *>(chain_heavy_kernel), hipFuncAttributeMaxDynamicSharedMemorySize,
                            (int)heavy_lds_bytes(kHeavyCap[5])) != hipSuccess) return -1;
    if (hipEventRecord(fork, st) != hipSuccess) return -1;
    for (int i = 0; i < 5; ++i)
        if (hipStreamWaitEvent(aux[i], fork, 0) != hipSuccess) return -1;
    unsigned long long *htk = A.ctr->heavy_tickets;
    chain_heavy_kernel<<<(unsigned)cu_count, 64, heavy_lds_bytes(kHeavyCap[5]), st>>>(A, &A.ctr->n_heavy, kHeavyCap[4], kHeavyCap[5], htk + 5);
    chain_heavy_kernel<<<(unsigned)(cu_count * 4), 64, heavy_lds_bytes(kHeavyCap[4]), aux[1]>>>(A, &A.ctr->n_heavy, kHeavyCap[3], kHeavyCap[4], htk + 4);
    chain_heavy_kernel<<<(unsigned)(cu_count * 7), 64, heavy_lds_bytes(kHeavyCap[3]), aux[2]>>>(A, &A.ctr->n_heavy, kHeavyCap[2], kHeavyCap[3], htk + 3);
    chain_heavy_kernel<<<(unsigned)(cu_count * 12), 64, heavy_lds_bytes(kHeavyCap[2]), aux[0]>>>(A, &A.ctr->n_heavy, kHeavyCap[1], kHeavyCap[2], htk + 2);
    chain_heavy_kernel<<<(unsigned)(cu_count * 16), 64, heavy_lds_bytes(kHeavyCap[1]), aux[3]>>>(A, &A.ctr->n_heavy, kHeavyCap[0], kHeavyCap[1], htk + 1);
    chain_heavy_kernel<<<(unsigned)(cu_count * 24), 64, heavy_lds_bytes(kHeavyCap[0]), aux[4]>>>(A, &A.ctr->n_heavy, 0, kHeavyCap[0], htk + 0);
    for (int i = 0; i < 5; ++i) {
        if (hipEventRecord(join[i], aux[i]) != hipSuccess) return -1;
        if (hipStreamWaitEvent(st, join[i], 0) != hipSuccess) return -1;
    }
    return 0;
}
#ifdef BWAMS_CHAIN_COUNT_TU
int launch_chain_counting(const ChainArgs &A, const uint32_t *n_seeds, int cu_count, hipStream_t st, hipStream_t *aux, hipEvent_t fork, hipEvent_t *join) {
    return launch_chain_t<true>(A, n_seeds, cu_count, st, aux, fork, join);
}
#else
int launch_chain_counting(const ChainArgs &A, const uint32_t *n_seeds, int cu_count, hipStream_t st, hipStream_t *aux, hipEvent_t fork, hipEvent_t *join);
int launch_chain(const ChainArgs &A, const uint32_t *n_seeds, int cu_count, hipStream_t st, hipStream_t *aux,
                 hipEvent_t fork, hipEvent_t *join, bool count) {
    return count ? launch_chain_counting(A, n_seeds, cu_count, st, aux, fork, join) : launch_chain_t<false>(A, n_seeds, cu_count, st, aux, fork, join);
}
void launch_chain_emit(const ChainArgs &A, const int64_t *chain_off, const int64_t *seed_off, bwams_chain_t *chains,
                       bwams_chain_seed_t *seeds, hipStream_t st) {
    if (A.nseq <= 0) return;
    chain_emit_kernel<<<(unsigned)((A.nseq * 16 + 255) / 256), 256, 0, st>>>(A, chain_off, seed_off, chains, seeds);
}

int launch_flt_sort_test(const int64_t *w, int n, int mode, int32_t *order) {
    if (n < 0 || n > kFltTestN) return -1;
    std::vector<uint2> h((size_t)n + 1);
    for (int i = 0; i < n; ++i) h[i] = make_uint2((unsigned)w[i], (unsigned)i);
    DevBuf<uint2> d_in, d_scr;
    DevBuf<int32_t> d_ord;
    if (d_in.alloc(8 * (size_t)(n + 1)) != hipSuccess || d_scr.alloc(8 * (size_t)(n + 1)) != hipSuccess || d_ord.alloc(4 * (size_t)(n + 1)) != hipSuccess ||
        hipMemcpy(d_in.p, h.data(), 8 * (size_t)n, hipMemcpyHostToDevice) != hipSuccess) return -1;
    flt_sort_test_kernel<<<1, 64>>>(d_in.p, n, mode, d_ord.p, d_scr.p);
    if (hipDeviceSynchronize() != hipSuccess || hipMemcpy(order, d_ord.p, 4 * (size_t)n, hipMemcpyDeviceToHost) != hipSuccess) return -1;
    return 0;
}
#endif

}
```

Before: 10.43.

## Replace sorted chain-key array with pre-ranked seeds and LDS occupancy bitmap

Before chaining, the seeds of each read are ranked by reference position with an in-LDS bitonic sort. Chain lookup becomes a predecessor query on a two-level occupancy bitmap indexed by seed rank, replacing the binary search and shift-insert into a sorted key array. Weight extraction now walks the bitmap in rank order instead of reading a sorted cid array. This trades per-insert O(n) shifts for an upfront sort per read plus extra LDS for the bitmap, which may lower occupancy for the larger classes.

```diff
diff --git a/bwa-mem-scale_amd/csrc/api_chain.hip b/bwa-mem-scale_amd/csrc/api_chain.hip
--- a/bwa-mem-scale_amd/csrc/api_chain.hip
+++ b/bwa-mem-scale_amd/csrc/api_chain.hip
@@ -194,6 +194,10 @@
     BWAMS_HIP(hipMemsetAsync(&b->d_ctr.p->chain_redo, 0, 23 * sizeof(unsigned long long), st));
     const bool count_ch = knobs().chain_count != 0;
     if (count_ch) BWAMS_HIP(hipMemsetAsync(b->d_ctr.p->dbg + 61, 0, 4 * sizeof(unsigned long long), st));
+#ifdef BWAMS_CHAINDBG
+    BWAMS_HIP(hipMemsetAsync(b->d_ctr.p->dbg + 32, 0, 29 * sizeof(unsigned long long), st));
+    BWAMS_HIP(hipMemsetAsync(b->d_ctr.p->dbg + 65, 0, 7 * sizeof(unsigned long long), st));
+#endif
     BWAMS_HIP(hipMemsetAsync(&b->d_ctr.p->chain_overflow, 0, 29 * sizeof(unsigned long long), st));
     if ((sv.one_smem_quirk ? sv.n_smem <= 1 : sv.n_smem <= 0) || n_sa == 0) {
         BWAMS_HIP(hipMemsetAsync(s->ch.n_kept.p, 0, (size_t)n1 * 4, st));
@@ -231,8 +235,8 @@
             fprintf(stderr, "[bwams_chain_run] chaining wave tier, per class: reads / mean us / longest us / wave-ms:");
             for (int c = 0; c < 8; ++c) fprintf(stderr, "  %s %llu / %.0f / %.0f / %.1f", cn[c], d[32 + 3 * c], d[32 + 3 * c] ? d[33 + 3 * c] * 1e-2 / d[32 + 3 * c] : 0.0, d[34 + 3 * c] * 1e-2, d[33 + 3 * c] * 1e-5);
             fprintf(stderr, "\n");
-            fprintf(stderr, "[bwams_chain_run] wave tier phases, G cycles: preamble %.2f chaining %.2f weights+copy %.2f (sort %.2f filter %.2f: all reads); reads %llu seeds %llu; passes %llu settling %llu seeds (%llu new chains), %llu seeds one by one%s; pass parts, G cycles: batch prologue %.2f search %.2f record+test %.2f settle %.2f commit %.2f one-by-one %.2f\n",
-                    d[56] / 1e9, d[57] / 1e9, d[58] / 1e9, d[8] / 1e9, d[9] / 1e9, d[59], d[60], count_ch ? d[61] : 0ull, count_ch ? d[63] : 0ull,
+            fprintf(stderr, "[bwams_chain_run] wave tier phases, G cycles: preamble %.2f ranking sort %.2f chaining (sort included) %.2f weights+copy %.2f (sort %.2f filter %.2f: all reads); reads %llu seeds %llu; passes %llu settling %llu seeds (%llu new chains), %llu seeds one by one%s; pass parts, G cycles: batch prologue %.2f search %.2f record+test %.2f settle %.2f commit %.2f one-by-one %.2f\n",
+                    d[56] / 1e9, d[71] / 1e9, d[57] / 1e9, d[58] / 1e9, d[8] / 1e9, d[9] / 1e9, d[59], d[60], count_ch ? d[61] : 0ull, count_ch ? d[63] : 0ull,
                     count_ch ? d[64] : 0ull, count_ch ? d[62] : 0ull, count_ch ? "" : " (these four are counted under BWAMS_CHAIN_COUNT=1 only)", d[65] / 1e9, d[66] / 1e9, d[67] / 1e9, d[68] / 1e9, d[69] / 1e9, d[70] / 1e9);
 #endif
         }
diff --git a/bwa-mem-scale_amd/csrc/chain.hip b/bwa-mem-scale_amd/csrc/chain.hip
--- a/bwa-mem-scale_amd/csrc/chain.hip
+++ b/bwa-mem-scale_amd/csrc/chain.hip
@@ -1,5 +1,6 @@
 #include "common.h"
 #include "chain_kernels.h"
+#include "chain_slots.h"
 #include "wave_ops.h"
 #include "ksort.h"
 
@@ -30,10 +31,11 @@
 __host__ __device__ constexpr size_t lds_bytes(int K) { return (size_t)K * (sizeof(ChainRec) + 12) + 64; }
 constexpr int kClassS = 128, kClassM1 = 256, kClassM = 512, kClassL1 = 850, kClassL = 1700;
 constexpr int kClassM2 = 665, kClassL2 = 1275;
-static_assert(lds_bytes(kClassL) <= 160 * 1024, "class L must fit one CU's LDS");
 constexpr int kClassXL = 4096;
 constexpr int kClassXL2 = 13000;
 __host__ __device__ constexpr size_t lds_bytes_xl(int K) { return (size_t)K * 12 + 64; }
+static_assert(lds_bytes_xl(kClassXL2) + slot_bytes(kClassXL2) <= 160 * 1024 && lds_bytes(kClassL) + slot_bytes(kClassL) <= 160 * 1024, "with the bitmap too");
+__host__ __device__ constexpr size_t slot_offset(size_t n) { return (n + 7) & ~(size_t)7; }
 
 struct RidCache { int64_t lo, hi; int rid; };
 
@@ -205,8 +207,6 @@
         xi = ci;
     }
 }
-
-struct WPath { int32_t leaf; int16_t slot, n; bool ok; };
 
 __device__ __forceinline__ int32_t kbt_traverse(const ReadCtx &c, int32_t *out) {
     int32_t sx[16];
@@ -383,58 +383,63 @@
 
 #endif
 
-__device__ __forceinline__ int sarr_lower(const int64_t *key, int n, int64_t k, int lane, bool &eq) {
-    int base = 0;
-    if (n > 4096) {
-        const int nsc = (n + 4095) >> 12;
-        const unsigned long long ms = __ballot(lane < nsc && key[lane << 12] <= k);
-        if (!ms) { eq = false; return -1; }
-        base = (__popcll(ms) - 1) << 12;
-        key += base;
-        n = n - base < 4096 ? n - base : 4096;
-    }
-    const int nch = (n + 63) >> 6;
-    const unsigned long long mc = __ballot(lane < nch && key[lane << 6] <= k);
-    if (!mc) { eq = false; return -1; }
-    const int c = __popcll(mc) - 1;
-    const int i = (c << 6) + lane;
-    const int64_t my = i < n ? key[i] : 0;
-    const unsigned long long mk = __ballot(i < n && my <= k);
-    const int idx = base + (c << 6) + __popcll(mk) - 1;
-    eq = __ballot(i < n && my == k) != 0;
-    return idx;
-}
-__device__ __forceinline__ void sarr_insert(int64_t *key, int32_t *cid, int n, int at, int64_t k, int32_t id, int lane) {
-    for (int base = ((n - at) >> 6) << 6; base >= 0; base -= 64) {
-        const int i = at + base + lane;
-        const bool mv = i < n;
-        const int64_t kk = mv ? key[i] : 0;
-        const int32_t cc = mv ? cid[i] : 0;
-        if (mv) { key[i + 1] = kk; cid[i + 1] = cc; }
-    }
-    if (lane == 0) { key[at] = k; cid[at] = id; }
-}
-
+constexpr int kRankBits = 20;
+static_assert(kClassXL2 < (1 << kRankBits), "seed indices of the largest LDS class fit the sort key");
+__device__ __forceinline__ void rank_seeds(const int64_t *pos, int32_t cnt, int64_t *skey, int32_t *rank, int lane) {
+    unsigned long long *key = reinterpret_cast<unsigned long long *>(skey);
+    for (int32_t g = lane; g < cnt; g += 64) key[g] = ((unsigned long long)pos[g] << kRankBits) | (unsigned long long)(unsigned)g;
+    __syncthreads();
+    int P = 64;
+    while (P < cnt) P <<= 1;
+    for (int k = 2; k <= P; k <<= 1) {
+        for (int j = k >> 1; j > 0; j >>= 1) {
+            const bool flip = j == (k >> 1);
+            for (int c0 = 0; c0 < (P >> 1); c0 += 64) {
+                const int c = c0 + lane;
+                const int i = ((c & ~(j - 1)) << 1) | (c & (j - 1));
+                const int l = flip ? (i ^ (k - 1)) : i + j;
+                if (l < cnt) {
+                    const unsigned long long x = key[i], y = key[l];
+                    if (y < x) { key[i] = y; key[l] = x; }
+                }
+            }
+            __syncthreads();
+        }
+    }
+    for (int32_t s = lane; s < cnt; s += 64) {
+        const unsigned long long v = key[s];
+        rank[(int32_t)(v & ((1ull << kRankBits) - 1ull))] = s;
+        skey[s] = (int64_t)(v >> kRankBits);
+    }
+    __threadfence_block();
+    __syncthreads();
+}
+
+using gmem_i32 = __attribute__((address_space(1))) int32_t;
+using gmem_i64 = __attribute__((address_space(1))) long long;
+__device__ __forceinline__ long long ql_pack(int qbeg, int len) { return (long long)(((unsigned long long)(unsigned)len << 32) | (unsigned long long)(unsigned)qbeg); }
 struct SeedCtx {
     bool crec_hbm;
     const int64_t *pos;
-    int32_t *s_next;
-    int2 *s_ql;
+    gmem_i32 *s_next;
+    gmem_i64 *s_ql;
     ChainRec *crec;
-    int64_t *s_key;
+    const int64_t *s_key;
     int32_t *s_cid;
+    uint64_t *bm, *sm;
+    const int32_t *rank;
 };
-__device__ __forceinline__ bool chain_seed_one(const ChainArgs &A, const SeedCtx &S, int &n_keys, int32_t g, int64_t rbeg, int rid, int qbeg,
+__device__ __forceinline__ bool chain_seed_one(const ChainArgs &A, const SeedCtx &S, int &n_keys, int32_t g, int64_t rbeg, int rk, int rid, int qbeg,
                                                int slen, int lane) {
     const bool wr = lane == 0;
     const int64_t l_pac = A.bns.l_pac;
     bool to_add = true, eq = false;
-    int idx = -1;
     if (n_keys) {
-        idx = sarr_lower(S.s_key, n_keys, rbeg, lane, eq);
+        const int idx = slot_pred(S.bm, S.sm, rk);
         if (idx >= 0) {
             const int32_t lower = S.s_cid[idx];
             const int64_t fr = S.s_key[idx];
+            eq = fr == rbeg;
             ChainRec ch = S.crec[lower];
             const int64_t lr = ch.last_rbeg;
             const int64_t qend = ch.last_qbeg + ch.last_len, rend = lr + ch.last_len;
@@ -444,7 +449,7 @@
             else {
                 const int64_t x = qbeg - ch.last_qbeg, y = rbeg - lr;
                 if (y >= 0 && x - y <= A.opt.w && y - x <= A.opt.w && x - ch.last_len < A.opt.max_chain_gap && y - ch.last_len < A.opt.max_chain_gap) {
-                    if (wr) { S.s_ql[g] = make_int2(qbeg, slen); S.s_next[g] = -1; S.s_next[ch.last_idx] = g; }
+                    if (wr) { S.s_ql[g] = ql_pack(qbeg, slen); S.s_next[g] = -1; S.s_next[ch.last_idx] = g; }
                     if (qbeg >= ch.endq) ch.wq += slen; else if (qbeg + slen > ch.endq) ch.wq += qbeg + slen - ch.endq;
                     ch.endq = (uint16_t)((int)ch.endq > qbeg + slen ? (int)ch.endq : qbeg + slen);
                     if (rbeg >= ch.endr) ch.wr += slen; else if (rbeg + slen > ch.endr) ch.wr += (int)(rbeg + slen - ch.endr);
@@ -457,16 +462,17 @@
         }
     }
     if (to_add) {
-        if (n_keys && eq) return false;
+        if (eq) return false;
         if (wr) {
-            S.s_ql[g] = make_int2(qbeg, slen); S.s_next[g] = -1;
+            S.s_ql[g] = ql_pack(qbeg, slen); S.s_next[g] = -1;
             ChainRec ch;
             ch.last_rbeg = rbeg; ch.endr = rbeg + slen;
             ch.first_qbeg = (uint16_t)qbeg; ch.last_qbeg = (uint16_t)qbeg; ch.last_len = (uint16_t)slen; ch.endq = (uint16_t)(qbeg + slen);
             ch.rid = rid; ch.n = 1; ch.first_idx = g; ch.last_idx = g; ch.wq = slen; ch.wr = slen;
             S.crec[n_keys] = ch;
-        }
-        sarr_insert(S.s_key, S.s_cid, n_keys, n_keys ? idx + 1 : 0, rbeg, n_keys, lane);
+            slot_set(S.bm, S.sm, rk);
+            S.s_cid[rk] = n_keys;
+        }
         ++n_keys;
     }
     return true;
@@ -497,6 +503,7 @@
         const int32_t g = gb + lane;
         bool pend = g < cnt;
         const int64_t rbeg = pend ? S.pos[g] : 0;
+        const int rk = pend ? S.rank[g] : 0;
         int qbeg = 0, slen = 0;
         if (sm_regs) {
             int k = 0;
@@ -532,7 +539,7 @@
         while ((mp = __ballot(pend)) != 0ull) {
             if (one_by_one) {
                 const int l0 = __builtin_ctzll(mp);
-                if (!chain_seed_one(A, S, n_keys, gb + l0, readlane64(rbeg, l0), __builtin_amdgcn_readlane(rid, l0), __builtin_amdgcn_readlane(qbeg, l0),
+                if (!chain_seed_one(A, S, n_keys, gb + l0, readlane64(rbeg, l0), __builtin_amdgcn_readlane(rk, l0), __builtin_amdgcn_readlane(rid, l0), __builtin_amdgcn_readlane(qbeg, l0),
                                     __builtin_amdgcn_readlane(slen, l0), lane)) return false;
                 if (lane == l0) pend = false;
                 if constexpr (COUNT) { if (lane == 0) atomicAdd(&A.ctr->dbg[62], 1ull); }
@@ -542,14 +549,7 @@
             }
             const int n = n_keys;
             int idx = -1;
-            if (n) {
-                int step = 1;
-                while ((step << 1) <= n) step <<= 1;
-                for (; step > 0; step >>= 1) {
-                    const int t = idx + step;
-                    if (pend && t < n && S.s_key[t] <= rbeg) idx = t;
-                }
-            }
+            if (n && pend) idx = slot_pred(S.bm, S.sm, rk);
             TQ(1)
             int64_t lo_key = INT64_MIN;
             int32_t lower = -1;
@@ -619,7 +619,7 @@
             const unsigned long long m_new = __ballot(com && act == NEW);
             if (__ballot(com && act == NEW && (eq || (displaced && best == rbeg)))) return false;
             if (com && act == MERGE) {
-                S.s_ql[g] = make_int2(qbeg, slen); S.s_next[g] = -1; S.s_next[ch.last_idx] = g;
+                S.s_ql[g] = ql_pack(qbeg, slen); S.s_next[g] = -1; S.s_next[ch.last_idx] = g;
                 if (qbeg >= ch.endq) ch.wq += slen; else if (qbeg + slen > ch.endq) ch.wq += qbeg + slen - ch.endq;
                 ch.endq = (uint16_t)((int)ch.endq > qbeg + slen ? (int)ch.endq : qbeg + slen);
                 if (rbeg >= ch.endr) ch.wr += slen; else if (rbeg + slen > ch.endr) ch.wr += (int)(rbeg + slen - ch.endr);
@@ -628,34 +628,18 @@
                 S.crec[lower] = ch;
             }
             if (m_new) {
-                const int m = __popcll(m_new);
-                const bool mine = com && act == NEW;
-                int min_idx = mine ? idx : n;
-                for (int d = 32; d >= 1; d >>= 1) { const int o = __shfl_xor(min_idx, d); min_idx = o < min_idx ? o : min_idx; }
-                for (int cb = n > 0 ? ((n - 1) >> 6) << 6 : -64; cb >= 0 && cb + 63 > min_idx; cb -= 64) {
-                    const int p = cb + lane;
-                    const bool mv = p < n;
-                    const int64_t kk = mv ? S.s_key[p] : 0;
-                    const int32_t cc = mv ? S.s_cid[p] : 0;
-                    int sh = __popcll(__ballot(mine && idx < cb));
-                    unsigned long long mm = __ballot(mine && idx >= cb && idx < cb + 64);
-                    while (mm) { const int i = __builtin_ctzll(mm); mm &= mm - 1; sh += __builtin_amdgcn_readlane(idx, i) < p ? 1 : 0; }
-                    if (mv && sh) { S.s_key[p + sh] = kk; S.s_cid[p + sh] = cc; }
-                }
-                int rank = 0;
-                { unsigned long long mm = m_new; while (mm) { const int i = __builtin_ctzll(mm); mm &= mm - 1; rank += __builtin_amdgcn_readlane(idx, i) < idx ? 1 : 0; } }
-                { unsigned long long mm = m_new & __ballot(shared); while (mm) { const int i = __builtin_ctzll(mm); mm &= mm - 1; rank += (__builtin_amdgcn_readlane(idx, i) == idx && readlane64(rbeg, i) < rbeg) ? 1 : 0; } }
-                if (mine) {
+                if (com && act == NEW) {
                     const int32_t cid = n + __popcll(m_new & below);
-                    S.s_ql[g] = make_int2(qbeg, slen); S.s_next[g] = -1;
+                    S.s_ql[g] = ql_pack(qbeg, slen); S.s_next[g] = -1;
                     ChainRec nc;
                     nc.last_rbeg = rbeg; nc.endr = rbeg + slen;
                     nc.first_qbeg = (uint16_t)qbeg; nc.last_qbeg = (uint16_t)qbeg; nc.last_len = (uint16_t)slen; nc.endq = (uint16_t)(qbeg + slen);
                     nc.rid = rid; nc.n = 1; nc.first_idx = g; nc.last_idx = g; nc.wq = slen; nc.wr = slen;
                     S.crec[cid] = nc;
-                    S.s_key[idx + 1 + rank] = rbeg; S.s_cid[idx + 1 + rank] = cid;
+                    slot_set(S.bm, S.sm, rk);
+                    S.s_cid[rk] = cid;
                 }
-                n_keys = n + m;
+                n_keys = n + __popcll(m_new);
             }
             if (com) pend = false;
             if constexpr (COUNT) {
@@ -677,7 +661,7 @@
 __host__ __device__ constexpr size_t heavy_lds_bytes(int cap);
 template <bool LDS, int CONT = 0, bool CREC_HBM = false, bool COUNT = false>
 __device__ __forceinline__ bool chain_read(const ChainArgs &A, int64_t r, int lane, int nl, Node *nodes, int32_t cap_nodes,
-                                           ChainRec *crec_w, int32_t cap_chains) {
+                                           ChainRec *crec_w, int32_t cap_chains, uint64_t *slots = nullptr) {
     const bool wr = lane == 0;
 #ifdef BWAMS_CHAINDBG
     const unsigned long long tp0 = __builtin_amdgcn_s_memtime();
@@ -738,9 +722,11 @@
     c.n_nodes = 0; c.n_keys = 0; c.overflow = false; c.wr = wr;
     int64_t *s_key = nullptr;
     int32_t *s_cid = nullptr;
+    uint64_t *s_bm = nullptr, *s_sm = nullptr;
     if constexpr (CONT == 1) {
         s_key = reinterpret_cast<int64_t *>(nodes);
         s_cid = reinterpret_cast<int32_t *>(s_key + cap_chains);
+        s_bm = slots; s_sm = slots + slot_words(cap_chains);
     } else c.root = new_node(c);
     RidCache rc;
     rc.lo = 0; rc.hi = -1; rc.rid = 0;
@@ -754,15 +740,37 @@
     const unsigned long long tp1 = __builtin_amdgcn_s_memtime();
 #endif
     if constexpr (CONT == 1) {
-        if (nl == 64 && A.seed_batch) {
-            SeedCtx S;
-            S.pos = pos; S.s_next = s_next; S.s_ql = s_ql; S.crec = crec; S.s_key = s_key; S.s_cid = s_cid; S.crec_hbm = CREC_HBM;
-            int nk = 0;
+        if (2 * l_pac >= (1ll << (63 - kRankBits))) return false;
+        int32_t *rank = A.f_kept + base;
+        for (int t = lane; t < slot_words(cnt); t += 64) s_bm[t] = 0ull;
+        if (lane < slot_sum_words(cap_chains)) s_sm[lane] = 0ull;
+        rank_seeds(pos, cnt, s_key, rank, lane);
+#ifdef BWAMS_CHAINDBG
+        if (wr) atomicAdd(&A.ctr->dbg[71], __builtin_amdgcn_s_memtime() - tp1);
+#endif
+        SeedCtx S;
+        S.pos = pos; S.s_next = (gmem_i32 *)s_next; S.s_ql = (gmem_i64 *)s_ql; S.crec = crec; S.s_key = s_key; S.s_cid = s_cid; S.crec_hbm = CREC_HBM;
+        S.bm = s_bm; S.sm = s_sm; S.rank = rank;
+        int nk = 0;
+        if (A.seed_batch) {
             if (!chain_seeds_batch<COUNT>(A, S, nk, sm, beg, end, base, cnt, rc, wb, lane)) return false;
-            c.n_keys = nk;
-        }
-    }
-    if (!(CONT == 1 && nl == 64 && A.seed_batch))
+        } else
+        for (int64_t i = beg; i < end; ++i) {
+            const int qbeg = (int)sm[i].m, slen = (int)sm[i].n + 1 - (int)sm[i].m;
+            const int32_t g0 = (int32_t)(A.sa_off[i] - base), g1 = (int32_t)(A.sa_off[i + 1] - base);
+            int64_t pos64 = 0;
+            int rank64 = 0;
+            for (int32_t g = g0; g < g1; ++g) {
+                const int j = (g - g0) & 63;
+                if (j == 0) { pos64 = g + lane < g1 ? pos[g + lane] : 0; rank64 = g + lane < g1 ? rank[g + lane] : 0; }
+                const int64_t rbeg = readlane64(pos64, j);
+                const int rid = A.bns.n_seqs <= 4096 ? intv2rid_w(A.bns, wb, rbeg, rbeg + slen, lane) : intv2rid(A.bns, rbeg, rbeg + slen, rc);
+                if (rid < 0) continue;
+                if (!chain_seed_one(A, S, nk, g, rbeg, __builtin_amdgcn_readlane(rank64, j), rid, qbeg, slen, lane)) return false;
+            }
+        }
+        c.n_keys = nk;
+    } else
     for (int64_t i = beg; i < end; ++i) {
         const int qbeg = (int)sm[i].m, slen = (int)sm[i].n + 1 - (int)sm[i].m;
         const int32_t g0 = (int32_t)(A.sa_off[i] - base), g1 = (int32_t)(A.sa_off[i + 1] - base);
@@ -779,18 +787,9 @@
                                                                : intv2rid(A.bns, rbeg, rbeg + slen, rc);
             if (rid < 0) continue;
             bool to_add = true;
-            WPath path;
-            path.ok = false;
             if (c.n_keys) {
                 int64_t fr = 0;
-                int32_t lower;
-                if constexpr (CONT == 1) {
-                    bool eq;
-                    const int idx = sarr_lower(s_key, c.n_keys, rbeg, lane, eq);
-                    lower = -1;
-                    if (idx >= 0) { lower = s_cid[idx]; fr = s_key[idx]; }
-                    path.slot = (int16_t)0; path.leaf = idx; path.ok = !eq;
-                } else lower = kbt_lower(c, rbeg, fr);
+                const int32_t lower = kbt_lower(c, rbeg, fr);
                 if (lower >= 0) {
                     ChainRec ch = crec[lower];
                     const int64_t lr = ch.last_rbeg;
@@ -826,11 +825,7 @@
                 ch.rid = rid; ch.n = 1; ch.first_idx = g; ch.last_idx = g; ch.wq = slen; ch.wr = slen;
                 const int32_t cid = c.n_keys;
                 if (wr) crec[cid] = ch;
-                if constexpr (CONT == 1) {
-                    if (c.n_keys && !path.ok) return false;
-                    sarr_insert(s_key, s_cid, c.n_keys, c.n_keys ? path.leaf + 1 : 0, rbeg, cid, lane);
-                    ++c.n_keys;
-                } else kbt_put(c, cid, rbeg);
+                kbt_put(c, cid, rbeg);
                 if (c.overflow) { if (wr) atomicAdd(&A.ctr->chain_overflow, 1ull); return true; }
             }
         }
@@ -841,21 +836,37 @@
 #endif
 
     int32_t *ord = A.f_first + base;
-    int32_t n_trav;
-    if constexpr (CONT == 1) {
-        n_trav = c.n_keys;
-        for (int32_t t = lane; t < n_trav; t += nl) ord[t] = s_cid[t];
-        __threadfence_block();
-    } else n_trav = kbt_traverse(c, ord);
+    int32_t n_trav = 0;
+    if constexpr (CONT == 0) n_trav = kbt_traverse(c, ord);
     uint2 *fl = A.flt + base;
     int n_chn = 0;
     if (nl == 64) {
         uint2 first = make_uint2(0u, 0u);
+        if constexpr (CONT == 1) {
+            bool have_first = false;
+            for (int32_t t0 = 0; t0 < cnt; t0 += 64) {
+                const unsigned long long occ = __ballot(((s_bm[t0 >> 6] >> lane) & 1ull) != 0ull);
+                if (!occ) continue;
+                const bool ok = ((occ >> lane) & 1ull) != 0ull;
+                const int32_t id = ok ? s_cid[t0 + lane] : 0;
+                const ChainRec *pc = &crec[id];
+                int w = pc->wr < pc->wq ? pc->wr : pc->wq;
+                w = w < (1 << 30) ? w : (1 << 30) - 1;
+                if (!have_first) {
+                    const int l0 = __builtin_ctzll(occ);
+                    first = make_uint2((unsigned)__builtin_amdgcn_readlane(w, l0), (unsigned)__builtin_amdgcn_readlane(id, l0));
+                    have_first = true;
+                }
+                const bool keep = ok && w >= A.opt.min_chain_weight;
+                const unsigned long long m = __ballot(keep);
+                if (keep) fl[n_chn + __popcll(m & ((1ull << lane) - 1ull))] = make_uint2((unsigned)w, (unsigned)id);
+                n_chn += __popcll(m);
+            }
+        } else
         for (int32_t t0 = 0; t0 < n_trav; t0 += 64) {
             const int32_t t = t0 + lane;
             const bool ok = t < n_trav;
-            int32_t id = 0;
-            if (ok) { if constexpr (CONT == 1) id = s_cid[t]; else id = ord[t]; }
+            const int32_t id = ok ? ord[t] : 0;
             const ChainRec *pc = &crec[id];
             int w = pc->wr < pc->wq ? pc->wr : pc->wq;
             w = w < (1 << 30) ? w : (1 << 30) - 1;
@@ -939,6 +950,7 @@
     const int64_t lo = lo_p ? (int64_t)*lo_p : 0, hi = (int64_t)*hi_p;
     ChainRec *l_crec = reinterpret_cast<ChainRec *>(l_mem);
     Node *l_nodes = reinterpret_cast<Node *>(l_mem + (size_t)(K > 0 ? K : 0) * sizeof(ChainRec));
+    uint64_t *l_slots = reinterpret_cast<uint64_t *>(l_mem + slot_offset(K < 0 ? (size_t)-K * 12 : (size_t)K * (sizeof(ChainRec) + 12)));
     for (;;) {
         const unsigned long long t = wave_ticket(ticket, 1ull);
         if (lo + (int64_t)t >= hi) break;
@@ -947,10 +959,10 @@
         const unsigned long long tk0 = wall_clock64();
 #endif
         if (K < 0) {
-            if (!chain_read<true, 1, true, COUNT>(A, r, lane, 64, reinterpret_cast<Node *>(l_mem), 0, nullptr, -K) && lane == 0)
+            if (!chain_read<true, 1, true, COUNT>(A, r, lane, 64, reinterpret_cast<Node *>(l_mem), 0, nullptr, -K, l_slots) && lane == 0)
                 A.redo[atomicAdd(&A.ctr->chain_redo, 1ull)] = (int32_t)r;
         } else if (K) {
-            if (!chain_read<true, 1, false, COUNT>(A, r, lane, 64, l_nodes, 0, l_crec, K) && lane == 0)
+            if (!chain_read<true, 1, false, COUNT>(A, r, lane, 64, l_nodes, 0, l_crec, K, l_slots) && lane == 0)
                 A.redo[atomicAdd(&A.ctr->chain_redo, 1ull)] = (int32_t)r;
         } else chain_read<false, 0, false, COUNT>(A, r, lane, 64, nullptr, 0, nullptr, 0);
         __syncthreads();
@@ -1259,21 +1271,21 @@
     if (A.nseq <= 0) return 0;
     unsigned long long *cls = A.ctr->chain_class, *tk = A.ctr->chain_ticket;
     if (hipFuncSetAttribute(reinterpret_cast<const void *>(chain_wave_kernel<COUNT>), hipFuncAttributeMaxDynamicSharedMemorySize,
-                            (int)lds_bytes_xl(kClassXL2)) != hipSuccess) return -1;
+                            (int)(lds_bytes_xl(kClassXL2) + slot_bytes(kClassXL2))) != hipSuccess) return -1;
     if (hipEventRecord(fork, st) != hipSuccess) return -1;
     for (int i = 0; i < 7; ++i)
         if (hipStreamWaitEvent(aux[i], fork, 0) != hipSuccess) return -1;
-    chain_wave_kernel<COUNT><<<(unsigned)cu_count, 64, lds_bytes_xl(kClassXL2), st>>>(A, cls + 9, cls + 6, tk + 9, -kClassXL2);
+    chain_wave_kernel<COUNT><<<(unsigned)cu_count, 64, lds_bytes_xl(kClassXL2) + slot_bytes(kClassXL2), st>>>(A, cls + 9, cls + 6, tk + 9, -kClassXL2);
     chain_wave_kernel<COUNT><<<(unsigned)(cu_count * 8), 64, 0, aux[0]>>>(A, nullptr, cls + 9, tk + 0, 0);
-    chain_wave_kernel<COUNT><<<(unsigned)cu_count, 64, lds_bytes_xl(kClassXL), aux[0]>>>(A, cls + 6, cls + 0, tk + 6, -kClassXL);
-    chain_wave_kernel<COUNT><<<(unsigned)cu_count, 64, lds_bytes(kClassL), aux[1]>>>(A, cls + 0, cls + 7, tk + 1, kClassL);
-    chain_wave_kernel<COUNT><<<(unsigned)(cu_count * 2), 64, lds_bytes(kClassL2), aux[5]>>>(A, cls + 7, cls + 1, tk + 7, kClassL2);
-    chain_wave_kernel<COUNT><<<(unsigned)(cu_count * 3), 64, lds_bytes(kClassL1), aux[2]>>>(A, cls + 1, cls + 8, tk + 2, kClassL1);
-    chain_wave_kernel<COUNT><<<(unsigned)(cu_count * 4), 64, lds_bytes(kClassM2), aux[6]>>>(A, cls + 8, cls + 2, tk + 8, kClassM2);
-    chain_wave_kernel<COUNT><<<(unsigned)(cu_count * 8), 64, lds_bytes(kClassM1), aux[2]>>>(A, cls + 3, cls + 4, tk + 4, kClassM1);
-    chain_wave_kernel<COUNT><<<(unsigned)(cu_count * 12), 64, lds_bytes(kClassS), aux[3]>>>(A, cls + 4, cls + 5, tk + 5, kClassS);
+    chain_wave_kernel<COUNT><<<(unsigned)cu_count, 64, lds_bytes_xl(kClassXL) + slot_bytes(kClassXL), aux[0]>>>(A, cls + 6, cls + 0, tk + 6, -kClassXL);
+    chain_wave_kernel<COUNT><<<(unsigned)cu_count, 64, lds_bytes(kClassL) + slot_bytes(kClassL), aux[1]>>>(A, cls + 0, cls + 7, tk + 1, kClassL);
+    chain_wave_kernel<COUNT><<<(unsigned)(cu_count * 2), 64, lds_bytes(kClassL2) + slot_bytes(kClassL2), aux[5]>>>(A, cls + 7, cls + 1, tk + 7, kClassL2);
+    chain_wave_kernel<COUNT><<<(unsigned)(cu_count * 3), 64, lds_bytes(kClassL1) + slot_bytes(kClassL1), aux[2]>>>(A, cls + 1, cls + 8, tk + 2, kClassL1);
+    chain_wave_kernel<COUNT><<<(unsigned)(cu_count * 4), 64, lds_bytes(kClassM2) + slot_bytes(kClassM2), aux[6]>>>(A, cls + 8, cls + 2, tk + 8, kClassM2);
+    chain_wave_kernel<COUNT><<<(unsigned)(cu_count * 8), 64, lds_bytes(kClassM1) + slot_bytes(kClassM1), aux[2]>>>(A, cls + 3, cls + 4, tk + 4, kClassM1);
+    chain_wave_kernel<COUNT><<<(unsigned)(cu_count * 12), 64, lds_bytes(kClassS) + slot_bytes(kClassS), aux[3]>>>(A, cls + 4, cls + 5, tk + 5, kClassS);
     chain_kernel<COUNT><<<(unsigned)((A.nseq + 63) / 64), 64, 0, aux[1]>>>(A, n_seeds);
-    chain_wave_kernel<COUNT><<<(unsigned)(cu_count * 5), 64, lds_bytes(kClassM), aux[5]>>>(A, cls + 2, cls + 3, tk + 3, kClassM);
+    chain_wave_kernel<COUNT><<<(unsigned)(cu_count * 5), 64, lds_bytes(kClassM) + slot_bytes(kClassM), aux[5]>>>(A, cls + 2, cls + 3, tk + 3, kClassM);
     for (int i = 0; i < 7; ++i) {
         if (hipEventRecord(join[i], aux[i]) != hipSuccess) return -1;
         if (hipStreamWaitEvent(st, join[i], 0) != hipSuccess) return -1;
diff --git a/bwa-mem-scale_amd/csrc/chain_slots.h b/bwa-mem-scale_amd/csrc/chain_slots.h
--- /dev/null
+++ b/bwa-mem-scale_amd/csrc/chain_slots.h
@@ -0,0 +1,42 @@
+#pragma once
+#include <cstddef>
+#include <cstdint>
+
+#if defined(__HIPCC__)
+#define BWAMS_SLOT_FN __host__ __device__ __forceinline__
+#else
+#define BWAMS_SLOT_FN inline
+#endif
+
+namespace bwams {
+
+constexpr int slot_words(int K) { return (K + 63) >> 6; }
+constexpr int slot_sum_words(int K) { return (slot_words(K) + 63) >> 6; }
+constexpr size_t slot_bytes(int K) { return 8 + 8 * (size_t)(slot_words(K) + slot_sum_words(K)); }
+
+BWAMS_SLOT_FN int slot_pred(const uint64_t *bm, const uint64_t *sm, int slot) {
+    int w = slot >> 6;
+    const uint64_t m = bm[w] & (~0ull >> (63 - (slot & 63)));
+    if (m) return (w << 6) + 63 - __builtin_clzll(m);
+    int sw = w >> 6;
+    uint64_t s = sm[sw] & ((1ull << (w & 63)) - 1ull);
+    while (!s) {
+        if (--sw < 0) return -1;
+        s = sm[sw];
+    }
+    w = (sw << 6) + 63 - __builtin_clzll(s);
+    return (w << 6) + 63 - __builtin_clzll(bm[w]);
+}
+
+BWAMS_SLOT_FN void slot_set(uint64_t *bm, uint64_t *sm, int slot) {
+    const int w = slot >> 6;
+#if defined(__HIP_DEVICE_COMPILE__)
+    atomicOr(reinterpret_cast<unsigned long long *>(&bm[w]), 1ull << (slot & 63));
+    atomicOr(reinterpret_cast<unsigned long long *>(&sm[w >> 6]), 1ull << (w & 63));
+#else
+    bm[w] |= 1ull << (slot & 63);
+    sm[w >> 6] |= 1ull << (w & 63);
+#endif
+}
+
+}
```

New measurement: 10.46 (median of 2 runs). About the same (+0.3%).
